# scychon/openmm_drudeNose

Measured on AMD Instinct MI355X. Metric: integrator steps/sec at 1M Drude pairs, higher is better.
Workload: dtype f64; 1 GPU; SWM4-NDP water box, 1000000 molecules = 5000000 particle slots, 1000000 Drude pairs, 1 temperature group (+ molecular-COM and Drude thermostats), TGNH mode, mixed precision, numNHChains=1, hard wall 0.02 nm, harness force call-out inside the timed region (harness_force: lattice); harness_force=lattice, precision=mixed, variant=resident, hipgraph=False, parallelism=particle-sharded x1 (whole molecules), one KE all-reduce per step, slots_per_gpu=5000000

## Files before the change

include/drude_tgnh.h:

```cpp
#ifndef DRUDE_TGNH_H_
#define DRUDE_TGNH_H_

#include <stdint.h>

#ifdef __cplusplus
extern "C" {
#endif

#define TGNH_ABI_VERSION 1

typedef int tgnh_status;
enum {
    TGNH_OK = 0,
    TGNH_ERR_ARG = -1,
    TGNH_ERR_GROUP_MISMATCH = -2,
    TGNH_ERR_HARDWALL = -3,
    TGNH_ERR_UNSUPPORTED = -4,
    TGNH_ERR_HIP = -5,
    TGNH_ERR_STATE = -6
};

enum { TGNH_MODE_DUALNH = 0,
       TGNH_MODE_TGNH = 1 };

enum { TGNH_PREC_SINGLE = 0,
       TGNH_PREC_MIXED = 1,
       TGNH_PREC_DOUBLE = 2 };

enum { TGNH_FLAG_DEFER_SCALE = 2 };
enum { TGNH_FLAG_WAVE_TILES = 8 };
enum { TGNH_FLAG_RESIDENT_STEP = 4 };

enum { TGNH_FLAG_TRUST_STATE_CHANGED = 16 };

enum { TGNH_FLAG_GATHER = 32 };

typedef struct tgnh_desc {
    uint32_t struct_size;
    int32_t mode;
    int32_t precision;
    int32_t flags;
    int32_t device;
    int32_t num_particles;
    int32_t padded_num_particles;
    int32_t num_pairs;
    int32_t num_groups;
    int32_t num_residues;
    int32_t num_constraints;
    int32_t has_cm_motion_remover;
    const double* mass;
    const int32_t* pair_drude;
    const int32_t* pair_parent;
    const int32_t* group;
    const int32_t* resid;
    const int32_t* constraint_i;
    const int32_t* constraint_j;
    double kB;
    double temperature, coupling_time;
    double drude_temperature, drude_coupling_time;
    double step_size;
    int32_t drude_steps_per_real_step;
    int32_t num_nh_chains;
    int32_t use_drude_nh_chains;
    int32_t use_com_temp_group;
    double max_drude_distance;
} tgnh_desc;

typedef struct tgnh_context* tgnh_handle;


typedef int (*tgnh_allreduce_fn)(void* buf, int count, void* stream, void* user);

const char* tgnh_last_error(void);
int tgnh_abi_version(void);

tgnh_status tgnh_create(const tgnh_desc* desc, tgnh_handle* out);
tgnh_status tgnh_destroy(tgnh_handle h);

tgnh_status tgnh_bind_buffers(tgnh_handle h, void* posq, void* posq_correction, void* velm,
                              const void* force, void* pos_delta);

tgnh_status tgnh_set_step_size(tgnh_handle h, double dt);
tgnh_status tgnh_set_drude_steps_per_real_step(tgnh_handle h, int n);
tgnh_status tgnh_set_max_drude_distance(tgnh_handle h, double d);

tgnh_status tgnh_get_local_dof_terms(tgnh_handle h, double* terms, int* count);
tgnh_status tgnh_set_global_dof_terms(tgnh_handle h, const double* terms, int count);
tgnh_status tgnh_set_allreduce(tgnh_handle h, tgnh_allreduce_fn fn, void* user);

#define TGNH_RCCL_ID_BYTES 128
tgnh_status tgnh_rccl_unique_id(void* id_out);
tgnh_status tgnh_rccl_init(tgnh_handle h, int world, int rank, const void* id);
tgnh_status tgnh_set_rccl_comm(tgnh_handle h, void* nccl_comm);
tgnh_status tgnh_rccl_shutdown(tgnh_handle h);
tgnh_status tgnh_set_resident_share(tgnh_handle h, int share);
tgnh_status tgnh_get_resident_work_groups(tgnh_handle h, int* per_compute_unit);
tgnh_status tgnh_get_step_path(tgnh_handle h, int* gather, const char** reason);
tgnh_status tgnh_get_resident_kernel(tgnh_handle h, int* which);

#define TGNH_XCHG_HANDLE_BYTES 64
tgnh_status tgnh_exchange_create(tgnh_handle h, int world, int rank, void* ipc_handle_out, void** mailbox_out);
tgnh_status tgnh_exchange_attach(tgnh_handle h, const void* ipc_handles);
tgnh_status tgnh_exchange_attach_pointers(tgnh_handle h, void* const* mailboxes);
tgnh_status tgnh_exchange_detach(tgnh_handle h);
tgnh_status tgnh_exchange_wait_stats(tgnh_handle h, void* stream, double* mean_us, double* max_us, int64_t* exchanges);

tgnh_status tgnh_step_begin(tgnh_handle h, void* stream);
tgnh_status tgnh_step_end(tgnh_handle h, void* stream);
tgnh_status tgnh_step_begin_kick(tgnh_handle h, void* stream);
tgnh_status tgnh_step_begin_move(tgnh_handle h, void* stream);
tgnh_status tgnh_step_end_kick(tgnh_handle h, void* stream);
tgnh_status tgnh_step_end_thermo(tgnh_handle h, void* stream);
tgnh_status tgnh_flush(tgnh_handle h, void* stream);
tgnh_status tgnh_note_replayed_steps(tgnh_handle h, int nsteps);
tgnh_status tgnh_get_pending_state(tgnh_handle h, uint32_t* bits);
tgnh_status tgnh_set_time(tgnh_handle h, double time, int64_t step_count);
tgnh_status tgnh_state_changed(tgnh_handle h);

tgnh_status tgnh_get_kinetic_energy(tgnh_handle h, int ke_sum_valid, void* stream, double* out);
tgnh_status tgnh_get_num_thermostats(tgnh_handle h, int* count);
tgnh_status tgnh_get_last_kinetic_energies(tgnh_handle h, void* stream, double* ke);
tgnh_status tgnh_get_last_scale_factors(tgnh_handle h, void* stream, double* scale);
tgnh_status tgnh_get_status_flags(tgnh_handle h, void* stream, uint32_t* flags);
tgnh_status tgnh_get_time(tgnh_handle h, double* time, int64_t* step_count);
tgnh_status tgnh_get_dof(tgnh_handle h, double* dof, double* nkt);

tgnh_status tgnh_get_thermostat_len(tgnh_handle h, int which, int* len);
tgnh_status tgnh_get_thermostat_state(tgnh_handle h, int which, void* stream, double* out);
tgnh_status tgnh_set_thermostat_state(tgnh_handle h, int which, void* stream, const double* in);

tgnh_status tgnh_get_topology_len(tgnh_handle h, int which, int* len);
tgnh_status tgnh_get_topology(tgnh_handle h, int which, int32_t* out);
tgnh_status tgnh_get_launch_bounds(tgnh_handle h, int32_t out[8]);

tgnh_status tgnh_compute_kinetic_energies(tgnh_handle h, void* stream);
tgnh_status tgnh_half_kick(tgnh_handle h, void* stream);

tgnh_status tgnh_harness_force(tgnh_handle h, const void* x0, double k_drude, double k_tether,
                               void* force_out, void* stream);
tgnh_status tgnh_harness_pack_sites(tgnh_handle h, const void* x0);
tgnh_status tgnh_harness_lattice_hint(tgnh_handle h, int mol_slots, int side, double spacing, const double* geom, int first_molecule);
tgnh_status tgnh_harness_sites_kind(tgnh_handle h, int* kind);
tgnh_status tgnh_run_steps(tgnh_handle h, int nsteps, void* stream);
tgnh_status tgnh_run_harness(tgnh_handle h, const void* x0, double k_drude, double k_tether,
                             int nsteps, void* stream);

tgnh_status tgnh_harness_set_clusters(tgnh_handle h, int n, const int32_t* atoms, const double* dist);
tgnh_status tgnh_harness_shake_positions(tgnh_handle h, double tol, void* stream);
tgnh_status tgnh_harness_shake_velocities(tgnh_handle h, double tol, void* stream);
tgnh_status tgnh_harness_set_virtual_sites(tgnh_handle h, int n, const int32_t* atoms, const double* weights);
tgnh_status tgnh_harness_virtual_sites(tgnh_handle h, void* stream);
tgnh_status tgnh_run_harness_constrained(tgnh_handle h, const void* x0, double k_drude, double k_tether,
                                         double tol, int nsteps, void* stream);

tgnh_status tgnh_harness_water_force(tgnh_handle h, double box, double cutoff, void* force_out, void* stream);
tgnh_status tgnh_harness_remove_cm_motion(tgnh_handle h, void* stream);

tgnh_status tgnh_timing_enable(tgnh_handle h, int on);
tgnh_status tgnh_timing_read(tgnh_handle h, int kernel, double* total_ms, int64_t* launches);
tgnh_status tgnh_algorithmic_bytes(tgnh_handle h, int kernel, double* bytes);

#ifdef __cplusplus
}
#endif
#endif
```

openmm_drudenose_amd/_lib.py:

```python
import ctypes as C
import os

HERE = os.path.dirname(os.path.abspath(__file__))
LIB_PATH = os.environ.get("TGNH_LIB") or os.path.join(HERE, "libdrudetgnh_hip.so")

TGNH_OK = 0
ERR_ARG, ERR_GROUP_MISMATCH, ERR_HARDWALL, ERR_UNSUPPORTED, ERR_HIP, ERR_STATE = -1, -2, -3, -4, -5, -6
MODE_DUALNH, MODE_TGNH = 0, 1
PREC_SINGLE, PREC_MIXED, PREC_DOUBLE = 0, 1, 2
FLAG_DEFER_SCALE, FLAG_RESIDENT_STEP, FLAG_WAVE_TILES, FLAG_TRUST_STATE_CHANGED, FLAG_GATHER = 2, 4, 8, 16, 32
KID_SKD, KID_KICK_KE, KID_SCALE, KID_KE, KID_CHAIN, KID_FORCE, KID_OTHER, KID_STEP = range(8)
KERNEL_NAMES = {KID_SKD: "scale+kick+drift", KID_KICK_KE: "kick+KE", KID_SCALE: "rescale", KID_KE: "KE",
                KID_CHAIN: "chain", KID_FORCE: "harness force", KID_OTHER: "other", KID_STEP: "resident step"}

c_i32p = C.POINTER(C.c_int32)
c_f64p = C.POINTER(C.c_double)


class TgnhDesc(C.Structure):
    _fields_ = [
        ("struct_size", C.c_uint32), ("mode", C.c_int32), ("precision", C.c_int32), ("flags", C.c_int32),
        ("device", C.c_int32), ("num_particles", C.c_int32), ("padded_num_particles", C.c_int32),
        ("num_pairs", C.c_int32), ("num_groups", C.c_int32), ("num_residues", C.c_int32),
        ("num_constraints", C.c_int32), ("has_cm_motion_remover", C.c_int32),
        ("mass", c_f64p), ("pair_drude", c_i32p), ("pair_parent", c_i32p), ("group", c_i32p), ("resid", c_i32p),
        ("constraint_i", c_i32p), ("constraint_j", c_i32p),
        ("kB", C.c_double), ("temperature", C.c_double), ("coupling_time", C.c_double),
        ("drude_temperature", C.c_double), ("drude_coupling_time", C.c_double), ("step_size", C.c_double),
        ("drude_steps_per_real_step", C.c_int32), ("num_nh_chains", C.c_int32),
        ("use_drude_nh_chains", C.c_int32), ("use_com_temp_group", C.c_int32),
        ("max_drude_distance", C.c_double),
    ]


ALLREDUCE_FN = C.CFUNCTYPE(C.c_int, C.c_void_p, C.c_int, C.c_void_p, C.c_void_p)

SIGNATURES = {
    "tgnh_last_error": (C.c_char_p, []),
    "tgnh_abi_version": (C.c_int, []),
    "tgnh_create": (C.c_int, [C.POINTER(TgnhDesc), C.POINTER(C.c_void_p)]),
    "tgnh_destroy": (C.c_int, [C.c_void_p]),
    "tgnh_bind_buffers": (C.c_int, [C.c_void_p] * 6),
    "tgnh_set_step_size": (C.c_int, [C.c_void_p, C.c_double]),
    "tgnh_set_drude_steps_per_real_step": (C.c_int, [C.c_void_p, C.c_int]),
    "tgnh_set_max_drude_distance": (C.c_int, [C.c_void_p, C.c_double]),
    "tgnh_get_local_dof_terms": (C.c_int, [C.c_void_p, c_f64p, C.POINTER(C.c_int)]),
    "tgnh_set_global_dof_terms": (C.c_int, [C.c_void_p, c_f64p, C.c_int]),
    "tgnh_set_allreduce": (C.c_int, [C.c_void_p, ALLREDUCE_FN, C.c_void_p]),
    "tgnh_rccl_unique_id": (C.c_int, [C.c_void_p]),
    "tgnh_rccl_init": (C.c_int, [C.c_void_p, C.c_int, C.c_int, C.c_void_p]),
    "tgnh_set_rccl_comm": (C.c_int, [C.c_void_p, C.c_void_p]),
    "tgnh_rccl_shutdown": (C.c_int, [C.c_void_p]),
    "tgnh_exchange_wait_stats": (C.c_int, [C.c_void_p, C.c_void_p, c_f64p, c_f64p, C.POINTER(C.c_int64)]),
    "tgnh_get_pending_state": (C.c_int, [C.c_void_p, C.POINTER(C.c_uint32)]),
    "tgnh_set_resident_share": (C.c_int, [C.c_void_p, C.c_int]),
    "tgnh_get_resident_work_groups": (C.c_int, [C.c_void_p, C.POINTER(C.c_int)]),
    "tgnh_get_resident_kernel": (C.c_int, [C.c_void_p, C.POINTER(C.c_int)]),
    "tgnh_get_step_path": (C.c_int, [C.c_void_p, C.POINTER(C.c_int), C.POINTER(C.c_char_p)]),
    "tgnh_exchange_create": (C.c_int, [C.c_void_p, C.c_int, C.c_int, C.c_void_p, C.POINTER(C.c_void_p)]),
    "tgnh_exchange_attach": (C.c_int, [C.c_void_p, C.c_char_p]),
    "tgnh_exchange_attach_pointers": (C.c_int, [C.c_void_p, C.POINTER(C.c_void_p)]),
    "tgnh_exchange_detach": (C.c_int, [C.c_void_p]),
    "tgnh_step_begin": (C.c_int, [C.c_void_p, C.c_void_p]),
    "tgnh_step_end": (C.c_int, [C.c_void_p, C.c_void_p]),
    "tgnh_step_begin_kick": (C.c_int, [C.c_void_p, C.c_void_p]),
    "tgnh_step_begin_move": (C.c_int, [C.c_void_p, C.c_void_p]),
    "tgnh_step_end_kick": (C.c_int, [C.c_void_p, C.c_void_p]),
    "tgnh_step_end_thermo": (C.c_int, [C.c_void_p, C.c_void_p]),
    "tgnh_flush": (C.c_int, [C.c_void_p, C.c_void_p]),
    "tgnh_state_changed": (C.c_int, [C.c_void_p]),
    "tgnh_note_replayed_steps": (C.c_int, [C.c_void_p, C.c_int]),
    "tgnh_set_time": (C.c_int, [C.c_void_p, C.c_double, C.c_int64]),
    "tgnh_get_kinetic_energy": (C.c_int, [C.c_void_p, C.c_int, C.c_void_p, c_f64p]),
    "tgnh_get_num_thermostats": (C.c_int, [C.c_void_p, C.POINTER(C.c_int)]),
    "tgnh_get_last_kinetic_energies": (C.c_int, [C.c_void_p, C.c_void_p, c_f64p]),
    "tgnh_get_last_scale_factors": (C.c_int, [C.c_void_p, C.c_void_p, c_f64p]),
    "tgnh_get_status_flags": (C.c_int, [C.c_void_p, C.c_void_p, C.POINTER(C.c_uint32)]),
    "tgnh_get_time": (C.c_int, [C.c_void_p, c_f64p, C.POINTER(C.c_int64)]),
    "tgnh_get_dof": (C.c_int, [C.c_void_p, c_f64p, c_f64p]),
    "tgnh_get_thermostat_len": (C.c_int, [C.c_void_p, C.c_int, C.POINTER(C.c_int)]),
    "tgnh_get_thermostat_state": (C.c_int, [C.c_void_p, C.c_int, C.c_void_p, c_f64p]),
    "tgnh_set_thermostat_state": (C.c_int, [C.c_void_p, C.c_int, C.c_void_p, c_f64p]),
    "tgnh_get_topology_len": (C.c_int, [C.c_void_p, C.c_int, C.POINTER(C.c_int)]),
    "tgnh_get_topology": (C.c_int, [C.c_void_p, C.c_int, c_i32p]),
    "tgnh_get_launch_bounds": (C.c_int, [C.c_void_p, c_i32p]),
    "tgnh_compute_kinetic_energies": (C.c_int, [C.c_void_p, C.c_void_p]),
    "tgnh_half_kick": (C.c_int, [C.c_void_p, C.c_void_p]),
    "tgnh_harness_force": (C.c_int, [C.c_void_p, C.c_void_p, C.c_double, C.c_double, C.c_void_p, C.c_void_p]),
    "tgnh_harness_pack_sites": (C.c_int, [C.c_void_p, C.c_void_p]),
    "tgnh_harness_lattice_hint": (C.c_int, [C.c_void_p, C.c_int, C.c_int, C.c_double, c_f64p, C.c_int]),
    "tgnh_harness_sites_kind": (C.c_int, [C.c_void_p, C.POINTER(C.c_int)]),
    "tgnh_run_harness": (C.c_int, [C.c_void_p, C.c_void_p, C.c_double, C.c_double, C.c_int, C.c_void_p]),
    "tgnh_run_steps": (C.c_int, [C.c_void_p, C.c_int, C.c_void_p]),
    "tgnh_harness_set_clusters": (C.c_int, [C.c_void_p, C.c_int, c_i32p, c_f64p]),
    "tgnh_harness_shake_positions": (C.c_int, [C.c_void_p, C.c_double, C.c_void_p]),
    "tgnh_harness_shake_velocities": (C.c_int, [C.c_void_p, C.c_double, C.c_void_p]),
    "tgnh_harness_set_virtual_sites": (C.c_int, [C.c_void_p, C.c_int, c_i32p, c_f64p]),
    "tgnh_harness_virtual_sites": (C.c_int, [C.c_void_p, C.c_void_p]),
    "tgnh_run_harness_constrained": (C.c_int, [C.c_void_p, C.c_void_p, C.c_double, C.c_double, C.c_double, C.c_int, C.c_void_p]),
    "tgnh_harness_water_force": (C.c_int, [C.c_void_p, C.c_double, C.c_double, C.c_void_p, C.c_void_p]),
    "tgnh_harness_remove_cm_motion": (C.c_int, [C.c_void_p, C.c_void_p]),
    "tgnh_timing_enable": (C.c_int, [C.c_void_p, C.c_int]),
    "tgnh_timing_read": (C.c_int, [C.c_void_p, C.c_int, c_f64p, C.POINTER(C.c_int64)]),
    "tgnh_algorithmic_bytes": (C.c_int, [C.c_void_p, C.c_int, c_f64p]),
}

_lib = None


def load():
    global _lib
    if _lib is not None:
        return _lib
    if not os.path.exists(LIB_PATH):
        raise RuntimeError(
            f"{LIB_PATH} is missing: build it with `python -m openmm_drudenose_amd.build` "
            "(hipcc --offload-arch=gfx950). There is no CPU fallback for the integrator path.")
    try:
        import torch
    except ImportError:
        pass
    lib = C.CDLL(LIB_PATH)
    for name, (res, args) in SIGNATURES.items():
        if os.environ.get("TGNH_LIB") and not hasattr(lib, name):
            continue
        fn = getattr(lib, name)
        fn.restype = res
        fn.argtypes = args
    _lib = lib
    return lib
```

openmm_drudenose_amd/csrc/tgnh_context.h:

```cpp
#ifndef TGNH_CONTEXT_H_
#define TGNH_CONTEXT_H_

#include <map>
#include <string>
#include <vector>

#include "tgnh_internal.h"

void tgnh_set_error(const std::string& msg);

namespace tgnh {
template <typename T> class DeviceBuf {
    T* p_ = nullptr;
    bool pinned_ = false;
public:
    DeviceBuf() = default;
    DeviceBuf(DeviceBuf&& o) noexcept : p_(o.p_), pinned_(o.pinned_) { o.p_ = nullptr; }
    ~DeviceBuf() { reset(); }
    void reset() { if (p_) (void)(pinned_ ? hipHostFree(p_) : hipFree(p_)); p_ = nullptr; }
    hipError_t alloc(size_t n, bool zero = false, unsigned ext_flags = 0) {
        reset(); pinned_ = false;
        void* p = nullptr;
        hipError_t e = ext_flags ? hipExtMallocWithFlags(&p, sizeof(T) * n, ext_flags) : hipMalloc(&p, sizeof(T) * n);
        if (e != hipSuccess) return e;
        p_ = static_cast<T*>(p);
        return zero ? hipMemset(p_, 0, sizeof(T) * n) : hipSuccess;
    }
    hipError_t alloc_pinned(size_t n) { reset(); pinned_ = true; return hipHostMalloc(reinterpret_cast<void**>(&p_), sizeof(T) * n, hipHostMallocDefault); }
    hipError_t upload(const T* src, size_t n) {
        hipError_t e = alloc(n ? n : 1);
        return e != hipSuccess || !n ? e : hipMemcpy(p_, src, sizeof(T) * n, hipMemcpyHostToDevice);
    }
    hipError_t upload(const std::vector<T>& v) { return upload(v.data(), v.size()); }
    T* get() const { return p_; }
    operator T*() const { return p_; }
};
typedef DeviceBuf<unsigned char> DeviceBytes;
}

struct tgnh_context {
    tgnh_desc d;
    int device = 0;
    bool host_only = false;
    struct Topology {
        std::vector<double> mass;
        std::vector<int> pair_drude, pair_parent, group, resid, normal;
        std::vector<int> res_count, res_first;
        std::vector<int> tile_start, tile_res;
        std::vector<int2> res_entries;
        std::vector<int> big_first, big_count;
        int num_big = 0, num_tiles = 0;
        std::vector<uint32_t> meta;
        std::vector<int2> wave_tile;
        std::vector<uint32_t> wmeta;
        std::vector<uint32_t> tile_pat, wtile_pat;
        std::vector<uint32_t> pattern, wpattern;
        int num_wtiles = 0;
        tgnh::DeviceBuf<uint32_t> d_meta, d_wmeta, d_tile_pat, d_pattern, d_wpattern;
        tgnh::DeviceBuf<int> d_tile_start, d_tile_res;
        tgnh::DeviceBuf<int2> d_res_table, d_wave_tile, d_big_table;
        tgnh::DeviceBytes d_big_com;
    } topo;
    struct Gather {
        bool generic = false;
        bool chain = false;
        std::string reason;
        std::vector<int2> res_table;
        std::vector<int> resid, partner;
        int com_lanes = 64;
        tgnh::DeviceBuf<int> d_group, d_resid, d_partner;
        tgnh::DeviceBuf<int2> d_res_table;
        tgnh::DeviceBytes d_com;
        tgnh::DeviceBuf<double> d_scratch;
    } gather;
    struct Thermostat {
        std::vector<double> h_state;
        std::vector<double> local_terms, global_terms;
        std::vector<double> dof, nkbt;
        double realkbT = 0, drudekbT = 0;
        tgnh::ChainLayout L{};
        tgnh::DeviceBuf<double> d_partials;
        tgnh::DeviceBuf<double> d_state;
        tgnh::DeviceBuf<double> d_stage;
        tgnh::DeviceBuf<double> d_scalar;
    } thermo;
    struct LaunchConfig {
        int grid = 0, gb = 1;
        int num_cus = 256, grid_override = 0;
        std::map<int, int> grid_cache;
        bool alternate_sweeps = true;
        int inline_sum_rows = tgnh::CHAIN_INLINE_SUM_ROWS;
        bool inline_sum_all = false;
        bool carry_ok = false;
        bool inline_chain = false;
        bool wave_ke = false;
        int resident_grid[5][2] = {{0, 0}, {0, 0}, {0, 0}, {0, 0}, {0, 0}};
        int resident_share = 1;
        int wresident_per_cu = 0, wresident_grid = 0;
        int resident_per_cu = 0;
    } cfg;
    struct Owed {
        bool end_pending = false;
        bool scale_pending = false;
        bool kick_pending = false;
        bool first_half_done = false;
        bool chain_pending = false;
        bool sum_pending = false;
        bool xwait_pending = false;
        bool stage_pending = false;
        bool ke_carry = false;
        bool chain_pending_twice = false;
        bool carry_pending = false;
        bool tail_summed = false;
        bool end_folded = false;
        bool g_com_fresh = false;
        enum : uint32_t { BIT_SWEEP_REVERSE = 1u << 8 };
        uint32_t bits() const {
            return end_pending | scale_pending << 1 | kick_pending << 2 | first_half_done << 3 | chain_pending << 4 | sum_pending << 5 |
                   xwait_pending << 6 | stage_pending << 7 | ke_carry << 9;
        }
        void chain_ran() { chain_pending = sum_pending = xwait_pending = carry_pending = false; }
        void velocities_current() { scale_pending = kick_pending = false; }
        void end_half_deferred(bool kick) { scale_pending = first_half_done = true; kick_pending = kick; }
        void resident_settled() { end_pending = first_half_done = false; velocities_current(); chain_pending = sum_pending = xwait_pending = false; }
        void thermostat_reset() { end_pending = first_half_done = false; velocities_current(); chain_pending = stage_pending = carry_pending = ke_carry = false; }
    } owed;
    struct Run {
        double time = 0;
        int64_t step_count = 0;
        int sweep_reverse = 0;
        int ke_parts = 0;
    } run;
    struct Bound {
        void *posq = nullptr, *posq_corr = nullptr, *velm = nullptr, *pos_delta = nullptr;
        const void* force = nullptr;
    } bound;
    struct Status {
        tgnh::DeviceBuf<uint32_t> d_word;
        tgnh::DeviceBuf<uint32_t> h_seen;
        int failed_code = 0;
        std::string failed;
    } status;
    struct Meeting {
        tgnh::DeviceBuf<unsigned int> d_sync;
        tgnh::DeviceBuf<unsigned long long> d_rows;
        tgnh::DeviceBuf<unsigned long long> self_box;
        tgnh::DeviceBuf<unsigned long long> d_self_misc;
        tgnh::XchgArgs self_x{};
    } meet;
    struct Exchange {
        tgnh_allreduce_fn allreduce = nullptr;
        void* allreduce_user = nullptr;
        void* rccl_comm = nullptr;
        bool rccl_owned = false;
        tgnh::XchgArgs args{};
        bool on = false;
        int world = 0, rank = 0;
        tgnh::DeviceBuf<unsigned long long> mailbox;
        tgnh::DeviceBuf<unsigned long long*> d_peers;
        std::vector<void*> opened;
        tgnh::DeviceBuf<unsigned long long> d_seq;
        tgnh::DeviceBuf<unsigned int> d_dead;
        tgnh::DeviceBuf<unsigned long long> d_stat;
        void close_peers() { for (void* p : opened) (void)hipIpcCloseMemHandle(p); opened.clear(); }
        ~Exchange() { close_peers(); }
    } xchg;
    struct Harness {
        tgnh::DeviceBuf<int4> d_cl_atoms, d_vs_atoms;
        tgnh::DeviceBuf<double> d_cl_dist, d_vs_w;
        int num_clusters = 0, num_sites = 0;
        tgnh::DeviceBuf<uint8_t> d_sflag;
        tgnh::DeviceBuf<uint32_t> d_sbase;
        tgnh::DeviceBytes d_sites;
        int lat_k = 0, lat_side = 0, lat_mol0 = 0;
        double lat_spacing = 0;
        std::vector<double> lat_geom;
        bool lat_on = false;
        tgnh::DeviceBuf<unsigned char> d_lat_tab;
        tgnh::DeviceBytes d_g_x0;
    } harness;
    struct Timing {
        bool on = false;
        int only = -1;
        struct Ev { hipEvent_t a, b; int kid; };
        std::vector<Ev> ev_pool;
        size_t ev_used = 0;
        double t_total[tgnh::KID_COUNT] = {0};
        int64_t t_count[tgnh::KID_COUNT] = {0};
        ~Timing() { for (auto& e : ev_pool) { (void)hipEventDestroy(e.a); (void)hipEventDestroy(e.b); } }
    } timing;
};

#endif
```

openmm_drudenose_amd/csrc/tgnh_internal.h:

```cpp
#ifndef TGNH_INTERNAL_H_
#define TGNH_INTERNAL_H_

#include <hip/hip_runtime.h>
#include <stdint.h>

#include "../../include/drude_tgnh.h"

namespace tgnh {

#ifndef TGNH_SPT
#define TGNH_SPT 2
#endif
#ifndef TGNH_TBLOCK
#define TGNH_TBLOCK 256
#endif
constexpr int BLOCK = 256;
constexpr int TBLOCK = TGNH_TBLOCK;
constexpr int SPT = TGNH_SPT;
constexpr int TILE_SLOTS = TBLOCK * SPT;
constexpr int TILE_RES = TILE_SLOTS / 2;
constexpr int GRID_CAP = 2048;
constexpr int MAX_GROUPS = 32;

constexpr uint32_t ROLE_NORMAL = 0, ROLE_DRUDE = 1, ROLE_PARENT = 2;
inline uint32_t pack_meta(uint32_t role, uint32_t group, int partner_off, uint32_t local_res) {
    return role | (group << 2) | ((uint32_t)(partner_off + 1024) << 10) | (local_res << 21);
}

constexpr int WAVE_SLOTS = 64;
constexpr int WBLOCK = 512;
inline uint32_t pack_wmeta(uint32_t role, uint32_t group, int partner_off, uint32_t pos_in_mol, uint32_t mol_slots_m1) {
    return role | (group << 2) | ((uint32_t)(partner_off + 64) << 10) | (pos_in_mol << 17) | (mol_slots_m1 << 23);
}

constexpr int PATTERN_WORDS = 64;

enum : int {
    OP_SCALE = 1,
    OP_KICK = 2,
    OP_DRIFT = 4,
    OP_KE = 8,
    OP_POSDELTA = 16,
    OP_MOVE = 32,
    OP_PREKICK = 64,
    OP_NOSTORE = 128
};

enum : int { KID_SKD = 0, KID_KICK_KE = 1, KID_SCALE = 2, KID_KE = 3, KID_CHAIN = 4, KID_FORCE = 5,
             KID_OTHER = 6, KID_STEP = 7, KID_COUNT = 8 };

struct ChainLayout {
    int mode, G, NT, C, use_drude_chains;
    int len_eta, len_etaDot, len_etaDotDot, len_etaMass;
    int off_eta, off_etaDot, off_etaDotDot, off_etaMass;
    int off_nkbt;
    int off_ke;
    int off_ke_red;
    int off_scale;
    int off_scale_a;
    int off_scale_b;
    int off_kesum;
    int off_ke_post;
    int total;
    int numTempGroup, idxMaxNHChains, iNumNHChains;
    int c1_shift, c1_mul, c1_add, c1_unused, c1_guard_below;
    int c1_quirk;
};

constexpr int XCHG_NT_PAD = 40;
constexpr int XCHG_CELL_U64 = 2;
constexpr int XCHG_MAX_WORLD = 16;
constexpr unsigned XCHG_SPIN_LIMIT = 1000000u;
constexpr unsigned CENSUS_SPIN_LIMIT = 20000u;
#ifndef TGNH_XCHG_REPLICAS
#define TGNH_XCHG_REPLICAS 32
#endif
constexpr int XCHG_REPLICAS = TGNH_XCHG_REPLICAS;
constexpr size_t XCHG_REPLICA_U64 =
    ((sizeof(unsigned long long) * 2 * (size_t)XCHG_MAX_WORLD * XCHG_NT_PAD * XCHG_CELL_U64 + 4095) / 4096 * 4096 + 256) / sizeof(unsigned long long);
constexpr size_t XCHG_MAILBOX_BYTES(int ) { return sizeof(unsigned long long) * XCHG_REPLICA_U64 * XCHG_REPLICAS; }

struct XchgArgs {
    int on;
    int world, rank;
    unsigned long long* const* peers;
    unsigned long long* mine;
    unsigned long long* seq;
    unsigned int* dead;
    unsigned int* status;
    unsigned long long* stat;
};

constexpr int CHAIN_INLINE_SUM_NT = 10;
constexpr int CHAIN_INLINE_SUM_ROWS = 256;

struct ChainArgs {
    ChainLayout L;
    XchgArgs x;
    int x_send, x_wait;
    double* st;
    uint32_t* status;
    const double* partials;
    int nparts;
    int nbig;
    const double* stage;
    int commit;
    int do_sum;
    int do_chain;
    int chain_twice;
    int lanes;
    int ke_carry;
    double dt;
    int S;
    double dtc, inv_dtc;
    double realkbT, drudekbT;
};

struct TileArgs {
    void* posq;
    void* posq_corr;
    void* velm;
    const long long* force;
    void* pos_delta;
    const uint32_t* meta;
    const int* tile_start;
    const int* tile_res;
    const int2* res_table;
    const void* big_com;
    const double* scale;
    double* partials;
    uint32_t* status;
    unsigned int* sync;
    int census;
    unsigned long long* rows;
    const int2* wave_tile;
    const uint32_t* wmeta;
    const uint32_t* tile_pat;
    const uint32_t* pattern;
    const uint32_t* wpattern;
    int num_wtiles;
    int tail_sum;
    double* ke_red;
    int num_tiles;
    int reverse;
    int padded;
    int num_groups;
    int use_com;
    int hardwall;
    double dt;
    double max_dist;
    double hw_scale;
    int chain_on;
    int sum_rows;
    int commit_len, commit_skip, commit_skip_n;
    const double* commit_src;
    double* commit_dst;
    int x_wait;
    const double* st_in;
    double* st_out;
    ChainArgs chain;
};

struct BigComArgs {
    const int2* table;
    int n;
    const void* velm;
    const long long* force;
    int padded;
    int kick;
    double dt;
    void* big_com;
    double* partials;
    int NT, G;
};

struct ForceArgs {
    const void* posq;
    const void* posq_corr;
    const void* x0;
    const uint32_t* meta;
    long long* force;
    int n, padded;
    int reverse;
    double k_drude, k_tether;
    const uint8_t* sflag;
    const uint32_t* sbase;
    const void* sites;
    int lat_k, lat_side, lat_mol0;
    double lat_spacing, lat_inv_k, lat_inv_side, lat_inv_side2;
    const unsigned char* lat_tab;
};
constexpr size_t LAT_TAB_BYTES = 64 + 64 * 3 * sizeof(double);

constexpr int GATHER_KE_ROWS = 1024;
constexpr int GATHER_MAX_NT = 2048;
struct GatherArgs {
    void* posq; void* posq_corr; void* velm; const long long* force; void* pos_delta;
    const int* group;
    const int* resid;
    const int2* res_table;
    const int* partner;
    void* com;
    const double* scale;
    double* partials;
    uint32_t* status;
    int n, padded, n_res, G, NT, use_com, hardwall, ops, kick_com;
    int com_lanes;
    double dt, max_dist, hw_scale;
};

#define TGNH_LAUNCH(...) do { (void)hipGetLastError(); hipLaunchKernelGGL(__VA_ARGS__); } while (0)

hipError_t launch_tile(int precision, int ops, int gb, const TileArgs& a, int grid, size_t lds, hipStream_t s);
int tile_blocks_per_cu(int precision, int ops, int gb, size_t lds, bool multi = false);
hipError_t launch_step(int precision, int gb, int kind, const TileArgs& a, int grid, size_t lds, hipStream_t s);
int step_blocks_per_cu(int precision, int gb, int kind, size_t lds);
int step_kind_ops2(int kind);
hipError_t launch_wstep(int precision, int gb, bool multi, const TileArgs& a, int grid, hipStream_t s);
int wstep_blocks_per_cu(int precision, int gb, bool multi);
hipError_t launch_wke(int precision, int ops, int gb, const TileArgs& a, int grid, hipStream_t s);
int wke_blocks_per_cu(int precision, int ops, int gb);
hipError_t launch_chain(const ChainArgs& a, hipStream_t s);
hipError_t launch_big_com(int precision, const BigComArgs& a, hipStream_t s);
hipError_t launch_force(int precision, const ForceArgs& a, hipStream_t s);
hipError_t launch_gather_com(int precision, const GatherArgs& a, hipStream_t s);
int gather_ke_grid(const GatherArgs& a);
hipError_t launch_gather_ke(int precision, const GatherArgs& a, int grid, hipStream_t s);
hipError_t launch_gather_rowsum(const double* partials, int nrows, int NT, double* ke_red, hipStream_t s);
hipError_t launch_gather_chain(const ChainArgs& a, double* scratch, hipStream_t s);
hipError_t launch_gather_update(int precision, const GatherArgs& a, hipStream_t s);
hipError_t launch_gather_force(int precision, const GatherArgs& a, const void* x0, long long* force, double k_drude, double k_tether, hipStream_t s);
constexpr int PLAIN_KE_PARTS = 2048;
hipError_t launch_plain_ke(int precision, const void* velm, const long long* force, int n, int padded,
                           double time_shift, double* out , hipStream_t s);
size_t tile_lds_bytes(int precision, int ops, bool hardwall, bool use_com);

}

#endif
```

openmm_drudenose_amd/csrc/tgnh_kernels.hip:

```cpp
#include "tgnh_tile_device.h"

#ifdef TGNH_TRACE
TGNH_TRACE_READERS(tgnh_debug_read_trace, tgnh_debug_clear_trace)
extern "C" int tgnh_debug_read_chain_trace(unsigned long long* out) {
    return (int)hipMemcpyFromSymbol(out, HIP_SYMBOL(tgnh::g_chain_trace), sizeof(unsigned long long) * 8);
}
#endif

namespace tgnh {


size_t tile_lds_bytes(int precision, int ops, bool hardwall, bool use_com) {
    (void)use_com;
    const size_t m4 = (precision == TGNH_PREC_SINGLE) ? 16 : 32;
    const bool hw = hardwall && (ops & (OP_DRIFT | OP_MOVE));
    size_t b = (size_t)(TBLOCK / 64) * (MAX_GROUPS + 2) * 8;
    if ((ops & (OP_SCALE | OP_KE)) || hw) b = m4 * (TILE_SLOTS + TILE_RES);
    if (hw) b += m4 * TILE_SLOTS;
    return b;
}

#ifndef TGNH_MINWAVES
#define TGNH_MINWAVES 1
#endif
// ... 644 lines not shown
    auto load = [&](const Bounds& b, WaveIn<PREC>& in) {
        const bool patterned = pw.of(a, (uint32_t)b.y >> 8, lane);
        wave_load<PREC, OPS>(a, b.ws, b.n, patterned, pw.word, lane, in);
    };
    if (w < nw) { bounds(w, b0); load(b0, A); }
    if (w + stride < nw) bounds(w + stride, b1);
    while (w < nw) {
        if (w + 2 * stride < nw) bounds(w + 2 * stride, b2);
        if (w + stride < nw) load(b1, B);
        work(A, b0);
        w += stride;
        if (w >= nw) break;
        if (w + 2 * stride < nw) bounds(w + 2 * stride, b0);
        if (w + stride < nw) load(b2, A);
        work(B, b1);
        w += stride;
        b1 = b0; b0 = b2;
    }
#pragma unroll
    for (int b = 0; b < GB; b++) ke_g[b] = wave_sum(ke_g[b]);
    ke_com = wave_sum(ke_com);
    ke_drude = wave_sum(ke_drude);
    if (lane == 0) {
#pragma unroll
        for (int b = 0; b < GB; b++) sred[wv][b] = ke_g[b];
        sred[wv][GB] = ke_com;
        sred[wv][GB + 1] = ke_drude;
    }
    __syncthreads();
    if (tid < GB + 2) {
        double t = 0.0;
#pragma unroll
        for (int k = 0; k < TBLOCK / 64; k++) t += sred[k][tid];
        const int b = tid < GB ? tid : G + (tid - GB);
        if (tid >= GB || tid < G) {
            if (a.tail_sum) {
                unsigned long long* cell = a.rows + row_word((int)blockIdx.x, 2 * b);
                const unsigned long long bits = (unsigned long long)__double_as_longlong(t), tg = (unsigned long long)(gen0 + 1u) << 32;
                __hip_atomic_store(cell, tg | (bits & 0xffffffffull), __ATOMIC_RELAXED, __HIP_MEMORY_SCOPE_SYSTEM);
                __hip_atomic_store(cell + 64, tg | (bits >> 32), __ATOMIC_RELAXED, __HIP_MEMORY_SCOPE_SYSTEM);
            } else a.partials[(size_t)blockIdx.x * (G + 2) + b] = t;
        }
    }
    if (a.tail_sum && blockIdx.x == 0) {
        __shared__ double s_tail[TBLOCK / 64][GB + 2];
        const int NT = G + 2;
        double acc[GB + 2];
#pragma unroll
        for (int b = 0; b < GB + 2; b++) acc[b] = 0.0;
        const bool ok = collect_rows<GB, false, TBLOCK>(a, tid, (int)gridDim.x, NT, (unsigned long long)(gen0 + 1u), acc);
        if (!ok) atomicOr(a.status, 16u);
#pragma unroll
        for (int b = 0; b < GB + 2; b++) {
            if (b < NT) {
                const double t = wave_sum(acc[b]);
                if (lane == 0) s_tail[wv][b] = t;
            }
        }
        const bool all_ok = __syncthreads_and(ok ? 1 : 0) != 0;
        if (tid < NT) {
            double t = 0.0;
#pragma unroll
            for (int k = 0; k < TBLOCK / 64; k++) t += s_tail[k][tid];
            a.ke_red[tid] = all_ok ? t : __longlong_as_double(0x7ff8000000000000ll);
        }
        if (tid == 0) a.sync[1] = gen0 + 1u;
    }
}



enum : int { STEP_DEFER = 0, STEP_PLAIN_BEGIN = 1, STEP_PLAIN_END = 2, STEP_SPLIT_BEGIN = 3, STEP_SPLIT_END = 4, STEP_KINDS = 5 };
constexpr int step_ops1(int kind) {
    return (kind == STEP_DEFER || kind == STEP_PLAIN_END) ? (OP_KICK | OP_KE | OP_NOSTORE) : OP_KE;
}
constexpr int step_ops2(int kind) {
    return kind == STEP_DEFER ? (OP_PREKICK | OP_SCALE | OP_KICK | OP_DRIFT)
         : kind == STEP_PLAIN_BEGIN ? (OP_SCALE | OP_KICK | OP_DRIFT)
         : kind == STEP_PLAIN_END ? (OP_PREKICK | OP_SCALE)
         : kind == STEP_SPLIT_BEGIN ? (OP_SCALE | OP_KICK | OP_POSDELTA)
         : OP_SCALE;
}

template <int PREC, int GB, int KIND>
__global__ __launch_bounds__(TBLOCK, TGNH_MINWAVES) void step_kernel(const TileArgs a) {
    typedef typename Prec<PREC>::mixed mixed;
    constexpr int STEP_OPS1 = step_ops1(KIND), STEP_OPS2 = step_ops2(KIND);
    __shared__ double s_scale[MAX_GROUPS + 2];
    __shared__ double s_part[TBLOCK / 64][CHAIN_INLINE_SUM_NT];
    __shared__ double s_x[64 + XCHG_MAX_WORLD * CHAIN_INLINE_SUM_NT];
    __shared__ int s_go;
    __shared__ unsigned s_gen;
    __shared__ unsigned long long s_seq1;
    extern __shared__ __attribute__((aligned(16))) char smem[];
    const int tid = threadIdx.x, G = a.num_groups, NT = G + 2;
    const int grid = (int)gridDim.x;
    const bool chain_wave = tid < 64;
    const int itg = tid & 63;
    if (a.census) {
        if (tid == 0) {
            __hip_atomic_fetch_add(&a.sync[2], 1u, __ATOMIC_RELAXED, __HIP_MEMORY_SCOPE_AGENT);
            unsigned n = 0;
            while (__hip_atomic_load(&a.sync[2], __ATOMIC_RELAXED, __HIP_MEMORY_SCOPE_AGENT) < gridDim.x && ++n < CENSUS_SPIN_LIMIT)
                __builtin_amdgcn_s_sleep(16);
            if (__hip_atomic_load(&a.sync[2], __ATOMIC_RELAXED, __HIP_MEMORY_SCOPE_AGENT) < gridDim.x) atomicOr(&a.sync[3], 1u);
        }
        return;
    }
    TileEnv<PREC, GB> e;
    e.init(a, smem, s_scale, OpsOf<STEP_OPS2>::POS && a.hardwall != 0);
    auto tile_of = [&](int tt) { return a.reverse ? a.num_tiles - 1 - tt : tt; };

    unsigned gen0 = 0;
    unsigned long long seq0 = 0;
    Chain1Regs creg{};
    if (chain_wave) {
        gen0 = __hip_atomic_load(&a.sync[1], __ATOMIC_RELAXED, __HIP_MEMORY_SCOPE_AGENT);
        seq0 = __hip_atomic_load(a.chain.x.seq, __ATOMIC_RELAXED, __HIP_MEMORY_SCOPE_AGENT);
        if (itg < NT) creg = chain1_load(a.chain, a.st_in, itg);
    }

    TRACE(0);
    TileIn<PREC> cur;
    int tt = blockIdx.x;
    TilePattern tp;
    tile_load<PREC, STEP_OPS1>(a, tile_of(tt), cur, tp);
    for (;;) {
        tile_body<PREC, STEP_OPS1, GB>(a, e, cur, 4);
        if (tt + grid >= a.num_tiles) break;
        tt += grid;
        tile_load<PREC, STEP_OPS1>(a, tile_of(tt), cur, tp);
    }
    const int tt_last = tt;
    TRACE(1);
    MeetShared sh{s_scale, s_part, s_x, &s_go, &s_gen, &s_seq1, nullptr};
    if (!step_meet<PREC, GB>(a, e, gen0, seq0, creg, sh, [&] { tile_load<PREC, STEP_OPS2, STEP_OPS1>(a, tile_of(tt_last), cur, tp); }))
        return;
    e.s_com = (mixed)s_scale[G]; e.s_drude = (mixed)s_scale[G + 1];
    TRACE(9);

    tt = tt_last;
    for (bool held = true;; held = false) {
        tile_body<PREC, STEP_OPS2, GB>(a, e, cur, 0, held);
        if (tt - grid < 0) break;
        tt -= grid;
        tile_load<PREC, STEP_OPS2>(a, tile_of(tt), cur, tp);
    }
    TRACE(15);
}


template <int PREC, int GB, bool MULTI = false>
__global__ __launch_bounds__(WBLOCK) void wstep_kernel(const TileArgs a) {
    typedef typename Prec<PREC>::mixed mixed;
    static_assert(GB > 0, "register bins only");
    __shared__ double s_scale[MAX_GROUPS + 2];
    __shared__ double s_part[WBLOCK / 64][CHAIN_INLINE_SUM_NT];
    __shared__ double s_x[64 + XCHG_MAX_WORLD * CHAIN_INLINE_SUM_NT];
    __shared__ int s_go;
    __shared__ unsigned s_gen;
    __shared__ unsigned long long s_seq1;
    __shared__ mixed s_img[WBLOCK / 64][7][WAVE_SLOTS];
    __shared__ double s_block[256];
    const int tid = threadIdx.x, lane = tid & 63, G = a.num_groups, NT = G + 2;
    const int wv = __builtin_amdgcn_readfirstlane(tid >> 6);
    const bool chain_wave = tid < 64;
    const int itg = tid & 63;
    if (a.census) {
        if (tid == 0) {
            __hip_atomic_fetch_add(&a.sync[2], 1u, __ATOMIC_RELAXED, __HIP_MEMORY_SCOPE_AGENT);
            unsigned n = 0;
            while (__hip_atomic_load(&a.sync[2], __ATOMIC_RELAXED, __HIP_MEMORY_SCOPE_AGENT) < gridDim.x && ++n < CENSUS_SPIN_LIMIT)
                __builtin_amdgcn_s_sleep(16);
            if (__hip_atomic_load(&a.sync[2], __ATOMIC_RELAXED, __HIP_MEMORY_SCOPE_AGENT) < gridDim.x) atomicOr(&a.sync[3], 1u);
        }
        return;
    }
    TileEnv<PREC, GB> e;
    e.tid = tid; e.G = G; e.smem = nullptr; e.wbins0 = nullptr; e.s_scale = s_scale;
    e.clear_ke();
    WaveStep<PREC, GB> ws(a, &e, s_scale, &s_img[wv][0][0], lane);
    typedef WaveBounds Bounds;
    auto bounds = [&](const int ww, Bounds& b) { ws.bounds(ww, b); };
    auto load_vf = [&](const Bounds& b, WStepIn<PREC>& in) { ws.load_vf(b, in); };
    auto load_x = [&](const Bounds& b, WStepIn<PREC>& in) { ws.load_x(b, in); };
    auto prepare = [&](WStepIn<PREC>& t, const Bounds& bd, const bool ke) { ws.template prepare<true>(t, bd, ke); };
    auto finish = [&](WStepIn<PREC>& t, const Bounds& bd) { ws.finish(t, bd); };
    auto wfence = [] { WaveStep<PREC, GB>::wfence(); };

    unsigned gen0 = 0;
    unsigned long long seq0 = 0;
    Chain1Regs creg{};
    if (chain_wave) {
        gen0 = __hip_atomic_load(&a.sync[1], __ATOMIC_RELAXED, __HIP_MEMORY_SCOPE_AGENT);
        seq0 = __hip_atomic_load(a.chain.x.seq, __ATOMIC_RELAXED, __HIP_MEMORY_SCOPE_AGENT);
        if (itg < NT && !(MULTI && a.chain.L.C > 1)) creg = chain1_load(a.chain, a.st_in, itg);
    }
    if (MULTI && a.chain.L.C > 1 && tid < a.chain.L.total) s_block[tid] = a.st_in[tid];

    const int nw = a.num_wtiles, stride = (int)gridDim.x * (WBLOCK / 64);

    TRACE(0);
    const int w0 = __builtin_amdgcn_readfirstlane((int)blockIdx.x * (WBLOCK / 64) + wv);
    const bool have = w0 < nw;
    int w = w0;
    Bounds b0{}, b1{};
    WStepIn<PREC> cur;
    if (have) {
        bounds(w, b0);
        if (w + stride < nw) bounds(w + stride, b1);
        load_vf(b0, cur);
    }
    while (have) {
#ifdef TGNH_TRACE
        if (w == w0) { asm volatile("s_waitcnt vmcnt(0)" ::: "memory"); TRACE(3); }
#endif
        prepare(cur, b0, true);
#ifdef TGNH_TRACE
        if (w == w0) TRACE(4);
#endif
        if (w + stride >= nw) break;
        wfence();
        w += stride;
        b0 = b1;
        if (w + stride < nw) bounds(w + stride, b1);
        load_vf(b0, cur);
    }
    const int w_last = w;
    TRACE(1);
    MeetShared sh{s_scale, s_part, s_x, &s_go, &s_gen, &s_seq1, s_block};
    if (!step_meet<PREC, GB, true, WBLOCK, MULTI>(a, e, gen0, seq0, creg, sh, [&] {
            if (have) {
                load_x(b0, cur);
                if (w_last - stride >= 0) bounds(w_last - stride, b1);
            }
        })) return;

    TRACE(9);
    if (have) {
        w = w_last;
        finish(cur, b0);
        TRACE(5);
        while (w - stride >= 0) {
            w -= stride;
            b0 = b1;
            if (w - stride >= 0) bounds(w - stride, b1);
            load_vf(b0, cur); load_x(b0, cur);
            prepare(cur, b0, false);
            finish(cur, b0);
        }
    }
    TRACE(15);
}

constexpr int CHAIN_LDS_DOUBLES = 2048;

__device__ __forceinline__ void chain_prologue(const ChainArgs& a, double (*sred)[MAX_GROUPS + 2], double* s_chain, double* s_ke) {
    const ChainLayout& L = a.L;
    const int NT = L.NT, tid = threadIdx.x, lane = tid & 63, wv = tid >> 6;
    double* st = a.st;
    if (a.commit) {
        for (int i = tid; i < L.total; i += BLOCK)
            if (i < L.off_ke_red || i >= L.off_ke_red + NT) st[i] = a.stage[i];
        __syncthreads();
    }
    if (a.do_sum) {
        constexpr int PER = GRID_CAP / BLOCK;
        double acc[MAX_GROUPS + 2];
#pragma unroll
        for (int b = 0; b < MAX_GROUPS + 2; b++) acc[b] = 0.0;
        if (NT <= 4) {
            double val[PER][4];
#pragma unroll
            for (int j = 0; j < PER; j++) {
                const int p = tid + j * BLOCK;
#pragma unroll
                for (int b = 0; b < 4; b++) val[j][b] = (p < a.nparts && b < NT) ? a.partials[(size_t)p * NT + b] : 0.0;
            }
#pragma unroll
            for (int j = 0; j < PER; j++)
#pragma unroll
                for (int b = 0; b < 4; b++) acc[b] += val[j][b];
        } else {
#pragma unroll
            for (int b = 0; b < MAX_GROUPS + 2; b++) {
                if (b < NT) {
                    double val[PER];
#pragma unroll
                    for (int j = 0; j < PER; j++) { const int p = tid + j * BLOCK; val[j] = p < a.nparts ? a.partials[(size_t)p * NT + b] : 0.0; }
#pragma unroll
                    for (int j = 0; j < PER; j++) acc[b] += val[j];
                }
            }
        }
        for (int p = tid; p < a.nbig; p += BLOCK) {
#pragma unroll
            for (int b = 0; b < MAX_GROUPS + 2; b++)
                if (b < NT) acc[b] += a.partials[((size_t)GRID_CAP + p) * NT + b];
        }
#pragma unroll
        for (int b = 0; b < MAX_GROUPS + 2; b++) {
            if (b < NT) {
                const double s = wave_sum(acc[b]);
                if (lane == 0) sred[wv][b] = s;
            }
        }
        __syncthreads();
        if (tid < NT) {
            double s = 0.0;
            for (int w = 0; w < BLOCK / 64; w++) s += sred[w][tid];
            st[L.off_ke_red + tid] = s;
            s_ke[tid] = s;
        }
        __syncthreads();
    } else if (tid < NT) {
        s_ke[tid] = st[chain_ke_src(a) + tid];
    }
    if (tid < NT && a.status && !a.ke_carry && s_ke[tid] != s_ke[tid]) atomicOr(a.status, 16u);
    if (a.x_send) xchg_send(a.x, NT, tid, BLOCK, s_chain, tid < NT ? s_ke[tid] : 0.0);
    if (a.x_wait) {
        __syncthreads();
        if (tid < 64) {
            const double tot = xchg_wait_sum(a.x, NT, tid, s_chain);
            if (tid < NT) { s_ke[tid] = tot; st[L.off_ke_red + tid] = tot; }
        }
        __syncthreads();
    }
}

__global__ __launch_bounds__(BLOCK) void rowsum_kernel(const ChainArgs a) {
    __shared__ double sred[BLOCK / 64][MAX_GROUPS + 2];
    __shared__ double s_chain[2 * XCHG_MAX_WORLD * XCHG_NT_PAD > 64 ? 2 * XCHG_MAX_WORLD * XCHG_NT_PAD : 64];
    __shared__ double s_ke[MAX_GROUPS + 2];
    chain_prologue(a, sred, s_chain, s_ke);
}

__global__ __launch_bounds__(BLOCK) void chain_kernel(const ChainArgs a) {
    __shared__ double sred[BLOCK / 64][MAX_GROUPS + 2];
    __shared__ double s_chain[CHAIN_LDS_DOUBLES];
    __shared__ double s_ke[MAX_GROUPS + 2];
    const ChainLayout& L = a.L;
    const int NT = L.NT, tid = threadIdx.x;
    double* st = a.st;
    CHAIN_TRACE(0);
    chain_prologue(a, sred, s_chain, s_ke);
    if (!a.do_chain) return;
    if (!a.do_sum) __syncthreads();
    CHAIN_TRACE(1);
    if (L.mode == TGNH_MODE_TGNH && L.C > 4 && L.C <= 16 && a.lanes) {
        chain_lanes_run(a, st, tid, BLOCK, s_ke);
        if (tid == 0) {
            double s = 0.0;
            for (int i = 0; i < NT; i++) s += s_ke[i];
            st[L.off_kesum] = 0.5 * s;
        }
    } else if (L.mode == TGNH_MODE_TGNH) {
        int itg = -1;
        if (tid < NT - 1) itg = tid;
        else if (tid == 64) itg = NT - 1;
        if (itg >= 0) {
            switch (L.C) {
                case 1: { Chain1Regs r = chain1_load(a, a.st, itg); r.ke = s_ke[itg]; chain1_run(a, r, a.st, true, nullptr, itg); } break;
                case 2: run_tgnh<2>(a, a.st, a.st, true, nullptr, itg, s_chain, s_ke[itg]); break;
                case 3: run_tgnh<3>(a, a.st, a.st, true, nullptr, itg, s_chain, s_ke[itg]); break;
                case 4: run_tgnh<4>(a, a.st, a.st, true, nullptr, itg, s_chain, s_ke[itg]); break;
                default: run_tgnh<0>(a, a.st, a.st, true, nullptr, itg, s_chain, s_ke[itg]); break;
            }
        }
        if (tid == 0) {
            double s = 0.0;
            for (int i = 0; i < NT; i++) s += s_ke[i];
            st[L.off_kesum] = 0.5 * s;
        }
    } else if (L.C == 1) {
        if (tid < 3) {
            Chain1Regs r = chain1_load(a, a.st, tid); r.ke = s_ke[tid];
            if (L.c1_quirk) chain1q_run(a, r, a.st, true, nullptr, tid);
            else chain1_run(a, r, a.st, true, nullptr, tid);
        }
        if (tid == 64) st[L.off_kesum] = 0.5 * (s_ke[0] + s_ke[2]);
    } else if (tid == 0) {
        switch (L.C) {
            case 1: run_dualnh<1>(a, a.st, a.st, true, nullptr, s_chain, s_ke[0], s_ke[1], s_ke[2]); break;
            case 2: run_dualnh<2>(a, a.st, a.st, true, nullptr, s_chain, s_ke[0], s_ke[1], s_ke[2]); break;
            case 3: run_dualnh<3>(a, a.st, a.st, true, nullptr, s_chain, s_ke[0], s_ke[1], s_ke[2]); break;
            case 4: run_dualnh<4>(a, a.st, a.st, true, nullptr, s_chain, s_ke[0], s_ke[1], s_ke[2]); break;
            default: run_dualnh<0>(a, a.st, a.st, true, nullptr, s_chain, s_ke[0], s_ke[1], s_ke[2]); break;
        }
    }
    CHAIN_TRACE(2);
}
template <int CC>
__global__ __launch_bounds__(BLOCK) void chain_long_kernel(const ChainArgs a) {
    __shared__ double sred[BLOCK / 64][MAX_GROUPS + 2];
    __shared__ double s_chain[2 * XCHG_MAX_WORLD * XCHG_NT_PAD > 64 ? 2 * XCHG_MAX_WORLD * XCHG_NT_PAD : 64];
    __shared__ double s_ke[MAX_GROUPS + 2];
    const ChainLayout& L = a.L;
    const int NT = L.NT, tid = threadIdx.x;
    chain_prologue(a, sred, s_chain, s_ke);
    if (!a.do_sum) __syncthreads();
    int itg = -1;
    if (tid < NT - 1) itg = tid;
    else if (tid == 64) itg = NT - 1;
    if (itg >= 0) run_tgnh<CC>(a, a.st, a.st, true, nullptr, itg, nullptr, s_ke[itg]);
    if (tid == 0) {
// ... 152 lines not shown
    if ((threadIdx.x & 63) == 0) sred[threadIdx.x >> 6] = e;
    __syncthreads();
    if (threadIdx.x == 0) {
        double s = 0.0;
        for (int w = 0; w < BLOCK / 64; w++) s += sred[w];
        out[1 + blockIdx.x] = s;
    }
}

__global__ __launch_bounds__(BLOCK) void plain_ke_sum_kernel(double* out, int nparts) {
    __shared__ double sred[BLOCK / 64];
    double e = 0.0;
    for (int i = threadIdx.x; i < nparts; i += BLOCK) e += out[1 + i];
    e = wave_sum(e);
    if ((threadIdx.x & 63) == 0) sred[threadIdx.x >> 6] = e;
    __syncthreads();
    if (threadIdx.x == 0) {
        double s = 0.0;
        for (int w = 0; w < BLOCK / 64; w++) s += sred[w];
        out[0] = 0.5 * s;
    }
}

typedef void (*tile_fn_t)(const TileArgs);

template <int PREC, int OPS>
static tile_fn_t tile_fn_gb(int gb) {
    if constexpr ((OPS & OP_KE) != 0) {
        if (gb == 0) return tile_kernel<PREC, OPS, 0>;
        if (gb <= 1) return tile_kernel<PREC, OPS, 1>;
        if (gb <= 4) return tile_kernel<PREC, OPS, 4>;
        return tile_kernel<PREC, OPS, 8>;
    } else {
        return tile_kernel<PREC, OPS, 1>;
    }
}

template <int PREC>
static tile_fn_t tile_fn_ops(int ops, int gb) {
    switch (ops) {
        case OP_KE: return tile_fn_gb<PREC, OP_KE>(gb);
        case OP_SCALE: return tile_fn_gb<PREC, OP_SCALE>(gb);
        case OP_SCALE | OP_KICK | OP_DRIFT: return tile_fn_gb<PREC, OP_SCALE | OP_KICK | OP_DRIFT>(gb);
        case OP_KICK | OP_KE: return tile_fn_gb<PREC, OP_KICK | OP_KE>(gb);
        case OP_KICK | OP_KE | OP_NOSTORE: return tile_fn_gb<PREC, OP_KICK | OP_KE | OP_NOSTORE>(gb);
        case OP_PREKICK | OP_SCALE | OP_KICK | OP_DRIFT: return tile_fn_gb<PREC, OP_PREKICK | OP_SCALE | OP_KICK | OP_DRIFT>(gb);
        case OP_PREKICK | OP_SCALE: return tile_fn_gb<PREC, OP_PREKICK | OP_SCALE>(gb);
        case OP_KICK: return tile_fn_gb<PREC, OP_KICK>(gb);
        case OP_SCALE | OP_KICK | OP_POSDELTA: return tile_fn_gb<PREC, OP_SCALE | OP_KICK | OP_POSDELTA>(gb);
        case OP_MOVE: return tile_fn_gb<PREC, OP_MOVE>(gb);
        default: return nullptr;
    }
}

static tile_fn_t tile_fn(int precision, int ops, int gb) {
    switch (precision) {
        case TGNH_PREC_SINGLE: return tile_fn_ops<TGNH_PREC_SINGLE>(ops, gb);
        case TGNH_PREC_MIXED: return tile_fn_ops<TGNH_PREC_MIXED>(ops, gb);
        case TGNH_PREC_DOUBLE: return tile_fn_ops<TGNH_PREC_DOUBLE>(ops, gb);
        default: return nullptr;
    }
}

template <int PREC> static tile_fn_t tile_fn_multi(int ops) {
    switch (ops) {
        case OP_SCALE: return tile_kernel<PREC, OP_SCALE, 1, true>;
        case OP_SCALE | OP_KICK | OP_DRIFT: return tile_kernel<PREC, OP_SCALE | OP_KICK | OP_DRIFT, 1, true>;
        case OP_PREKICK | OP_SCALE | OP_KICK | OP_DRIFT: return tile_kernel<PREC, OP_PREKICK | OP_SCALE | OP_KICK | OP_DRIFT, 1, true>;
        case OP_PREKICK | OP_SCALE: return tile_kernel<PREC, OP_PREKICK | OP_SCALE, 1, true>;
        case OP_SCALE | OP_KICK | OP_POSDELTA: return tile_kernel<PREC, OP_SCALE | OP_KICK | OP_POSDELTA, 1, true>;
        default: return nullptr;
    }
}
static tile_fn_t tile_fn_any(int precision, int ops, int gb, bool multi) {
    if (!multi) return tile_fn(precision, ops, gb);
    switch (precision) {
        case TGNH_PREC_SINGLE: return tile_fn_multi<TGNH_PREC_SINGLE>(ops);
        case TGNH_PREC_MIXED: return tile_fn_multi<TGNH_PREC_MIXED>(ops);
        case TGNH_PREC_DOUBLE: return tile_fn_multi<TGNH_PREC_DOUBLE>(ops);
        default: return nullptr;
    }
}

hipError_t launch_tile(int precision, int ops, int gb, const TileArgs& a, int grid, size_t lds, hipStream_t s) {
    tile_fn_t fn = tile_fn_any(precision, ops, gb, a.chain_on && a.chain.L.C > 1);
    if (!fn) return hipErrorInvalidValue;
    TGNH_LAUNCH(fn, dim3(grid), dim3(TBLOCK), lds, s, a);
    return hipGetLastError();
}

template <int PREC, int OPS> static tile_fn_t wke_fn_gb(int gb) {
    if (gb <= 1) return wke_kernel<PREC, OPS, 1>;
    if (gb <= 4) return wke_kernel<PREC, OPS, 4>;
    return wke_kernel<PREC, OPS, 8>;
}
template <int PREC> static tile_fn_t wke_fn_ops(int ops, int gb) {
    switch (ops) {
        case OP_KE: return wke_fn_gb<PREC, OP_KE>(gb);
        case OP_KICK | OP_KE: return wke_fn_gb<PREC, OP_KICK | OP_KE>(gb);
        case OP_KICK | OP_KE | OP_NOSTORE: return wke_fn_gb<PREC, OP_KICK | OP_KE | OP_NOSTORE>(gb);
        default: return nullptr;
    }
}
static tile_fn_t wke_fn(int precision, int ops, int gb) {
    if (gb == 0) return nullptr;
    switch (precision) {
        case TGNH_PREC_SINGLE: return wke_fn_ops<TGNH_PREC_SINGLE>(ops, gb);
        case TGNH_PREC_MIXED: return wke_fn_ops<TGNH_PREC_MIXED>(ops, gb);
        case TGNH_PREC_DOUBLE: return wke_fn_ops<TGNH_PREC_DOUBLE>(ops, gb);
        default: return nullptr;
    }
}
hipError_t launch_wke(int precision, int ops, int gb, const TileArgs& a, int grid, hipStream_t s) {
    tile_fn_t fn = wke_fn(precision, ops, gb);
    if (!fn) return hipErrorInvalidValue;
    TGNH_LAUNCH(fn, dim3(grid), dim3(TBLOCK), 0, s, a);
    return hipGetLastError();
}
int wke_blocks_per_cu(int precision, int ops, int gb) {
    tile_fn_t fn = wke_fn(precision, ops, gb);
    int n = 0;
    if (!fn || hipOccupancyMaxActiveBlocksPerMultiprocessor(&n, reinterpret_cast<const void*>(fn), TBLOCK, 0) != hipSuccess) return 0;
    return n;
}

typedef void (*step_fn_t)(const TileArgs);
template <int PREC, int KIND> static step_fn_t step_fn_gb(int gb) {
    if (gb <= 1) return step_kernel<PREC, 1, KIND>;
    if (gb <= 4) return step_kernel<PREC, 4, KIND>;
    return step_kernel<PREC, 8, KIND>;
}
template <int PREC> static step_fn_t step_fn_kind(int kind, int gb) {
    switch (kind) {
        case STEP_DEFER: return step_fn_gb<PREC, STEP_DEFER>(gb);
        case STEP_PLAIN_BEGIN: return step_fn_gb<PREC, STEP_PLAIN_BEGIN>(gb);
        case STEP_PLAIN_END: return step_fn_gb<PREC, STEP_PLAIN_END>(gb);
        case STEP_SPLIT_BEGIN: return step_fn_gb<PREC, STEP_SPLIT_BEGIN>(gb);
        case STEP_SPLIT_END: return step_fn_gb<PREC, STEP_SPLIT_END>(gb);
        default: return nullptr;
    }
}
static step_fn_t step_fn(int precision, int gb, int kind) {
    if (gb == 0) return nullptr;
    switch (precision) {
        case TGNH_PREC_SINGLE: return step_fn_kind<TGNH_PREC_SINGLE>(kind, gb);
        case TGNH_PREC_MIXED: return step_fn_kind<TGNH_PREC_MIXED>(kind, gb);
        case TGNH_PREC_DOUBLE: return step_fn_kind<TGNH_PREC_DOUBLE>(kind, gb);
        default: return nullptr;
    }
}
template <int PREC, bool MULTI> static step_fn_t wstep_fn_gb(int gb) {
    return gb <= 1 ? wstep_kernel<PREC, 1, MULTI> : gb <= 4 ? wstep_kernel<PREC, 4, MULTI> : wstep_kernel<PREC, 8, MULTI>;
}
static step_fn_t wstep_fn(int precision, int gb, bool multi) {
    if (gb == 0) return nullptr;
    switch (precision) {
        case TGNH_PREC_SINGLE: return multi ? wstep_fn_gb<TGNH_PREC_SINGLE, true>(gb) : wstep_fn_gb<TGNH_PREC_SINGLE, false>(gb);
        case TGNH_PREC_MIXED: return multi ? wstep_fn_gb<TGNH_PREC_MIXED, true>(gb) : wstep_fn_gb<TGNH_PREC_MIXED, false>(gb);
        case TGNH_PREC_DOUBLE: return multi ? wstep_fn_gb<TGNH_PREC_DOUBLE, true>(gb) : wstep_fn_gb<TGNH_PREC_DOUBLE, false>(gb);
        default: return nullptr;
    }
}
hipError_t launch_wstep(int precision, int gb, bool multi, const TileArgs& a, int grid, hipStream_t s) {
    step_fn_t fn = wstep_fn(precision, gb, multi);
    if (!fn) return hipErrorInvalidValue;
    TGNH_LAUNCH(fn, dim3(grid), dim3(WBLOCK), 0, s, a);
    return hipGetLastError();
}
int wstep_blocks_per_cu(int precision, int gb, bool multi) {
    step_fn_t fn = wstep_fn(precision, gb, multi);
    int n = 0;
    if (!fn || hipOccupancyMaxActiveBlocksPerMultiprocessor(&n, reinterpret_cast<const void*>(fn), WBLOCK, 0) != hipSuccess) return 0;
    return n;
}
int step_kind_ops2(int kind) { return step_ops2(kind); }
hipError_t launch_step(int precision, int gb, int kind, const TileArgs& a, int grid, size_t lds, hipStream_t s) {
    step_fn_t fn = step_fn(precision, gb, kind);
    if (!fn) return hipErrorInvalidValue;
    TGNH_LAUNCH(fn, dim3(grid), dim3(TBLOCK), lds, s, a);
    return hipGetLastError();
}
int step_blocks_per_cu(int precision, int gb, int kind, size_t lds) {
    step_fn_t fn = step_fn(precision, gb, kind);
    int n = 0;
    if (!fn || hipOccupancyMaxActiveBlocksPerMultiprocessor(&n, reinterpret_cast<const void*>(fn), TBLOCK, lds) != hipSuccess) return 0;
    return n;
}

int tile_blocks_per_cu(int precision, int ops, int gb, size_t lds, bool multi) {
    tile_fn_t fn = tile_fn_any(precision, ops, gb, multi);
    int n = 0;
    if (!fn || hipOccupancyMaxActiveBlocksPerMultiprocessor(&n, reinterpret_cast<const void*>(fn), TBLOCK, lds) != hipSuccess) return 0;
    return n;
}

hipError_t launch_chain(const ChainArgs& a, hipStream_t s) {
    if (!a.do_chain) TGNH_LAUNCH(rowsum_kernel, dim3(1), dim3(BLOCK), 0, s, a);
    else if (a.L.mode == TGNH_MODE_TGNH && a.L.C > 4 && a.L.C <= 16 && !a.lanes) {
        switch (a.L.C) {
#define TGNH_LONG(c) case c: TGNH_LAUNCH(chain_long_kernel<c>, dim3(1), dim3(BLOCK), 0, s, a); break;
            TGNH_LONG(5) TGNH_LONG(6) TGNH_LONG(7) TGNH_LONG(8) TGNH_LONG(9) TGNH_LONG(10) TGNH_LONG(11) TGNH_LONG(12)
            TGNH_LONG(13) TGNH_LONG(14) TGNH_LONG(15) TGNH_LONG(16)
#undef TGNH_LONG
        }
    }
    else if (a.L.mode == TGNH_MODE_DUALNH && a.L.C > 4 && a.L.C <= 16) {
        switch (a.L.C) {
#define TGNH_DLONG(c) case c: TGNH_LAUNCH(chain_dualnh_long_kernel<c>, dim3(1), dim3(BLOCK), 0, s, a); break;
            TGNH_DLONG(5) TGNH_DLONG(6) TGNH_DLONG(7) TGNH_DLONG(8) TGNH_DLONG(9) TGNH_DLONG(10) TGNH_DLONG(11) TGNH_DLONG(12)
            TGNH_DLONG(13) TGNH_DLONG(14) TGNH_DLONG(15) TGNH_DLONG(16)
#undef TGNH_DLONG
        }
    }
    else TGNH_LAUNCH(chain_kernel, dim3(1), dim3(BLOCK), 0, s, a);
#ifdef TGNH_TUNING
    static const int again = getenv("TGNH_CHAIN_REPEAT") ? atoi(getenv("TGNH_CHAIN_REPEAT")) : 0;
    for (int r = 0; r < again && a.do_chain; r++) { ChainArgs b = a; b.do_sum = 0; b.commit = 0; b.x_send = 0; b.x_wait = 0; TGNH_LAUNCH(chain_kernel, dim3(1), dim3(BLOCK), 0, s, b); }
#endif
    return hipGetLastError();
}

template <int PREC>
__global__ __launch_bounds__(BLOCK) void force_packed_kernel(const ForceArgs a) {
    typedef typename Prec<PREC>::real real;
    typedef typename Prec<PREC>::real4 real4;
    typedef typename Prec<PREC>::mixed mixed;
    const real4* __restrict__ posq = reinterpret_cast<const real4*>(a.posq);
    const float4* __restrict__ pcorr = reinterpret_cast<const float4*>(a.posq_corr);
    const real* __restrict__ sites = reinterpret_cast<const real*>(a.sites);
    const mixed kd = (mixed)a.k_drude, kt = (mixed)a.k_tether;
    const int lane = threadIdx.x & 63;
    const int nround = (a.n + gridDim.x * BLOCK - 1) / (gridDim.x * BLOCK);
    for (int rr = 0; rr < nround; rr++) {
        const int r = a.reverse ? nround - 1 - rr : rr;
        const int blk = a.reverse ? (int)gridDim.x - 1 - (int)blockIdx.x : (int)blockIdx.x;
        const int i = (r * gridDim.x + blk) * BLOCK + threadIdx.x;
        const bool in = i < a.n;
        uint32_t b = 0;
        real4 p = {}; float4 c = {};
        if (in) {
            b = a.sflag[i];
            p = posq[i];
            if (PREC == TGNH_PREC_MIXED) c = pcorr[i];
        }
        const bool tethered = (b & 4u) != 0;
        const unsigned long long before = __ballot(tethered) & ((1ull << lane) - 1ull);
        real s0 = 0, s1 = 0, s2 = 0;
        if (tethered) {
            const real* rec = sites + 3 * (size_t)(a.sbase[i >> 6] + (uint32_t)__popcll(before));
            s0 = rec[0]; s1 = rec[1]; s2 = rec[2];
        }
        mixed x = p.x, y = p.y, z = p.z;
        if (PREC == TGNH_PREC_MIXED) { x += (mixed)c.x; y += (mixed)c.y; z += (mixed)c.z; }
        const uint32_t role = b & 3u;
        int off = (int)(b >> 3) - 16;
        if (in && (b >> 3) == 0) off = (int)((a.meta[i] >> 10) & 2047u) - 1024;
        const int pl = lane + off;
        const int src = (pl >= 0 && pl < 64) ? pl : lane;
        mixed ox = __shfl(x, src, 64), oy = __shfl(y, src, 64), oz = __shfl(z, src, 64);
        mixed fx = 0, fy = 0, fz = 0;
        if (in) {
            if (tethered) { fx = -kt * (x - (mixed)s0); fy = -kt * (y - (mixed)s1); fz = -kt * (z - (mixed)s2); }
            if (role != ROLE_NORMAL) {
                if (src != pl) {
                    const int j = i + off;
                    const real4 q = posq[j];
                    ox = q.x; oy = q.y; oz = q.z;
                    if (PREC == TGNH_PREC_MIXED) { const float4 cq = pcorr[j]; ox += (mixed)cq.x; oy += (mixed)cq.y; oz += (mixed)cq.z; }
                }
                const bool is_d = role == ROLE_DRUDE;
                const mixed sgn = is_d ? (mixed)-1 : (mixed)1;
                const mixed sx = is_d ? x - ox : ox - x, sy = is_d ? y - oy : oy - y, sz = is_d ? z - oz : oz - z;
                fx += sgn * kd * sx; fy += sgn * kd * sy; fz += sgn * kd * sz;
            }
            a.force[i] = (long long)(fx * (mixed)4294967296.0);
            a.force[i + a.padded] = (long long)(fy * (mixed)4294967296.0);
            a.force[i + 2 * a.padded] = (long long)(fz * (mixed)4294967296.0);
        }
    }
}

template <int PREC>
__global__ __launch_bounds__(BLOCK) void force_lattice_kernel(const ForceArgs a) {
    typedef typename Prec<PREC>::real real;
    typedef typename Prec<PREC>::real4 real4;
    typedef typename Prec<PREC>::mixed mixed;
    __shared__ double s_geom[64 * 3];
    __shared__ unsigned char s_flag[64];
    const real4* __restrict__ posq = reinterpret_cast<const real4*>(a.posq);
    const float4* __restrict__ pcorr = reinterpret_cast<const float4*>(a.posq_corr);
    if (threadIdx.x < 64) s_flag[threadIdx.x] = a.lat_tab[threadIdx.x];
    if (threadIdx.x < 192) s_geom[threadIdx.x] = reinterpret_cast<const double*>(a.lat_tab + 64)[threadIdx.x];
    __syncthreads();
    const mixed kd = (mixed)a.k_drude, kt = (mixed)a.k_tether;
    const int lane = threadIdx.x & 63;
    const int nround = (a.n + gridDim.x * BLOCK - 1) / (gridDim.x * BLOCK);
    for (int rr = 0; rr < nround; rr++) {
        const int r = a.reverse ? nround - 1 - rr : rr;
        const int blk = a.reverse ? (int)gridDim.x - 1 - (int)blockIdx.x : (int)blockIdx.x;
        const int i = (r * gridDim.x + blk) * BLOCK + threadIdx.x;
        const bool in = i < a.n;
        real4 p = {}; float4 c = {};
        if (in) {
            p = posq[i];
            if (PREC == TGNH_PREC_MIXED) c = pcorr[i];
        }
        const int mloc = (int)(((double)i + 0.5) * a.lat_inv_k), pos = in ? i - mloc * a.lat_k : 0;
        const int mol = a.lat_mol0 + mloc;
        const uint32_t b = in ? s_flag[pos] : 0u;
        const bool tethered = (b & 4u) != 0;
        real s0 = 0, s1 = 0, s2 = 0;
        if (tethered) {
            const int ix = (int)(((double)mol + 0.5) * a.lat_inv_side2), rem = mol - ix * a.lat_side * a.lat_side;
            const int iy = (int)(((double)rem + 0.5) * a.lat_inv_side), iz = rem - iy * a.lat_side;
            s0 = (real)__dadd_rn(__dmul_rn((double)ix, a.lat_spacing), s_geom[3 * pos]);
            s1 = (real)__dadd_rn(__dmul_rn((double)iy, a.lat_spacing), s_geom[3 * pos + 1]);
            s2 = (real)__dadd_rn(__dmul_rn((double)iz, a.lat_spacing), s_geom[3 * pos + 2]);
        }
        mixed x = p.x, y = p.y, z = p.z;
        if (PREC == TGNH_PREC_MIXED) { x += (mixed)c.x; y += (mixed)c.y; z += (mixed)c.z; }
        const uint32_t role = b & 3u;
        const int off = (int)(b >> 3) - 16;
        const int pl = lane + off;
// ... 80 lines not shown
```

openmm_drudenose_amd/csrc/tgnh_lifecycle.cpp:

```cpp
#include <memory>

#include "tgnh_host.h"
#ifndef TGNH_MEETING_MEM
#define TGNH_MEETING_MEM hipDeviceMallocFinegrained
#endif

static thread_local std::string g_err;
extern "C" const char* tgnh_last_error(void) { return g_err.c_str(); }
extern "C" int tgnh_abi_version(void) { return TGNH_ABI_VERSION; }

void tgnh_set_error(const std::string& msg) { g_err = msg; }

static tgnh_status validate_desc(const tgnh_desc* d, bool* long_chain) {
    if (d->struct_size != sizeof(tgnh_desc)) return fail(TGNH_ERR_ARG, "tgnh_desc size mismatch (ABI)");
    if (d->mode != TGNH_MODE_DUALNH && d->mode != TGNH_MODE_TGNH) return fail(TGNH_ERR_ARG, "bad mode");
    if (d->precision < TGNH_PREC_SINGLE || d->precision > TGNH_PREC_DOUBLE) return fail(TGNH_ERR_ARG, "bad precision");
    if (d->num_particles < 1 || d->num_pairs < 0 || !d->mass || (d->num_pairs && (!d->pair_drude || !d->pair_parent)))
        return fail(TGNH_ERR_ARG, "bad particle / pair arrays");
    if (d->padded_num_particles < d->num_particles) return fail(TGNH_ERR_ARG, "padded_num_particles < num_particles");
    if (d->num_constraints < 0) return fail(TGNH_ERR_ARG, "negative num_constraints");
    if (3LL * d->padded_num_particles > 2147483647LL)
        return fail(TGNH_ERR_UNSUPPORTED, "more than 715 827 882 padded particle slots: the index into the third force plane leaves 32 bits");
    if (d->num_nh_chains < 1 || d->drude_steps_per_real_step < 1) return fail(TGNH_ERR_ARG, "numNHChains and drudeStepsPerRealStep must be >= 1");
    if (d->mode == TGNH_MODE_TGNH && (d->num_groups < 1 || d->num_residues < 1 || !d->group || !d->resid))
        return fail(TGNH_ERR_ARG, "TGNH mode needs temperature groups and residues");
    if (!(d->max_drude_distance >= 0)) return fail(TGNH_ERR_ARG, "setMaxDrudeDistance: Distance cannot be negative");
    if (d->flags & ~(uint32_t)(TGNH_FLAG_DEFER_SCALE | TGNH_FLAG_RESIDENT_STEP | TGNH_FLAG_WAVE_TILES | TGNH_FLAG_TRUST_STATE_CHANGED | TGNH_FLAG_GATHER))
        return fail(TGNH_ERR_ARG, "unknown bits in tgnh_desc.flags (a newer header than this library?)");
    if (d->mode == TGNH_MODE_DUALNH && d->num_pairs == 0)
        return fail(TGNH_ERR_UNSUPPORTED, "dualNH mode needs at least one Drude pair (the Reference platform does too)");
    if (!(d->step_size > 0) || !std::isfinite(d->step_size)) return fail(TGNH_ERR_ARG, "step size must be positive");
    *long_chain = false;
    {
        const long need = d->mode == TGNH_MODE_TGNH ? (long)(d->num_groups + 2) * (4L * d->num_nh_chains + 1)
                                                    : 4L * (2L * d->num_nh_chains + 4);
        if (d->num_nh_chains > (d->mode == TGNH_MODE_TGNH ? 16 : 4) && need > 2048) {
            if (d->mode != TGNH_MODE_TGNH) return fail(TGNH_ERR_UNSUPPORTED, "numNHChains too large for the on-device chain");
            *long_chain = true;
        }
    }
    return TGNH_OK;
}

static tgnh_status decide_policy(tgnh_context* c, const tgnh_desc* d, bool long_chain) {
    if (c->gather.generic) {
        c->d.flags &= ~(TGNH_FLAG_DEFER_SCALE | TGNH_FLAG_RESIDENT_STEP | TGNH_FLAG_TRUST_STATE_CHANGED | TGNH_FLAG_WAVE_TILES);
        c->gather.chain = c->d.mode == TGNH_MODE_TGNH && (c->thermo.L.NT > MAX_GROUPS + 2 || long_chain);
    }
    c->cfg.wave_ke = !c->gather.generic && !c->topo.wave_tile.empty() && c->cfg.gb != 0 &&
                 ((d->flags & TGNH_FLAG_WAVE_TILES) || (double)d->num_particles >= 0.9 * WAVE_SLOTS * (double)c->topo.num_wtiles);
#ifdef TGNH_TUNING
    if (const char* e = getenv("TGNH_WAVE_KE")) c->cfg.wave_ke = c->cfg.wave_ke && e[0] != '0';
#endif
    {
        bool inside = true;
        if (d->mode == TGNH_MODE_TGNH && d->use_com_temp_group) {
            std::vector<int> g0(d->num_residues, -1);
            for (int i = 0; i < d->num_particles && inside; i++) {
                if (c->topo.mass[i] == 0.0) continue;
                int& g = g0[c->topo.resid[i]];
                if (g == -1) g = c->topo.group[i];
                else if (g != c->topo.group[i]) inside = false;
            }
        }
        if ((c->d.flags & TGNH_FLAG_DEFER_SCALE) && !inside) return fail(TGNH_ERR_UNSUPPORTED, "DEFER_SCALE needs every molecule inside one temperature group");
        c->cfg.carry_ok = (c->d.flags & TGNH_FLAG_TRUST_STATE_CHANGED) && !(c->d.flags & TGNH_FLAG_DEFER_SCALE) && inside;
    }
    c->cfg.grid = GRID_CAP;
#ifdef TGNH_TUNING
    if (const char* e = getenv("TGNH_GRID")) { int g = atoi(e); if (g >= 1) c->cfg.grid_override = std::min(g, GRID_CAP); }
#endif
    {
        bool want = true;
        c->cfg.inline_sum_all = d->num_particles < 2000000;
#ifdef TGNH_TUNING
        if (const char* e = getenv("TGNH_INLINE_CHAIN")) want = e[0] != '0';
        if (const char* e4 = getenv("TGNH_INLINE_SUM_ROWS")) c->cfg.inline_sum_rows = atoi(e4);
        if (const char* e5 = getenv("TGNH_INLINE_SUM_ALL")) c->cfg.inline_sum_all = e5[0] != '0';
        if (const char* e3 = getenv("TGNH_ALTERNATE_SWEEPS")) c->cfg.alternate_sweeps = e3[0] != '0';
#endif
        int inline_multi_max = 2500000;
#ifdef TGNH_TUNING
        if (const char* e6 = getenv("TGNH_INLINE_MULTI_MAX")) inline_multi_max = atoi(e6);
#endif
        c->cfg.inline_chain = want && !c->gather.generic && (c->thermo.L.C == 1 || (c->thermo.L.C <= 4 && d->num_particles < inline_multi_max));
        if (c->thermo.L.total > 256 && c->thermo.L.C > 1) c->cfg.inline_chain = c->cfg.inline_chain && false;
    }
    return TGNH_OK;
}

static tgnh_status allocate(tgnh_context* c) {
    const size_t NT = c->thermo.L.NT;
    HIP_OK(c->thermo.d_partials.alloc((size_t)(c->cfg.grid + c->topo.num_big) * NT, true));
    HIP_OK(c->thermo.d_state.alloc(c->thermo.L.total));
    HIP_OK(c->thermo.d_stage.alloc(c->thermo.L.total));
    HIP_OK(c->status.d_word.alloc(1, true));
    HIP_OK(c->status.h_seen.alloc_pinned(1));
    *c->status.h_seen = 0;
    if (c->gather.chain && c->thermo.L.C > 4) HIP_OK(c->gather.d_scratch.alloc(NT * (4 * c->thermo.L.C + 1)));
    HIP_OK(c->thermo.d_scalar.alloc(1 + PLAIN_KE_PARTS));
    HIP_OK(c->meet.d_sync.alloc(4, true));
    const bool resident = (c->d.flags & TGNH_FLAG_RESIDENT_STEP) != 0;
    if (c->cfg.wave_ke || resident)
        HIP_OK(c->meet.d_rows.alloc(2 * (size_t)GRID_CAP * CHAIN_INLINE_SUM_NT, true, TGNH_MEETING_MEM));
    if (!resident) return TGNH_OK;
    HIP_OK(c->meet.self_box.alloc(XCHG_MAILBOX_BYTES(1) / sizeof(unsigned long long), true, TGNH_MEETING_MEM));
    HIP_OK(c->meet.d_self_misc.alloc(4, true));
    unsigned long long* const box = c->meet.self_box;
    HIP_OK(hipMemcpy(c->meet.d_self_misc + 2, &box, sizeof(box), hipMemcpyHostToDevice));
    c->meet.self_x = XchgArgs{};
    c->meet.self_x.on = 1; c->meet.self_x.world = 1; c->meet.self_x.rank = 0;
    c->meet.self_x.peers = reinterpret_cast<unsigned long long* const*>(c->meet.d_self_misc + 2);
    c->meet.self_x.mine = c->meet.self_box;
    c->meet.self_x.seq = c->meet.d_self_misc;
    c->meet.self_x.dead = reinterpret_cast<unsigned int*>(c->meet.d_self_misc + 1);
    c->meet.self_x.status = c->status.d_word;
    return TGNH_OK;
}

template <typename Launch> static tgnh_status census(tgnh_context* c, int per_cu_max, Launch&& launch, int* found) {
    for (int per_cu = std::min(per_cu_max, 8); per_cu >= 1 && !*found; per_cu--) {
        TileArgs a{};
        a.census = 1; a.sync = c->meet.d_sync;
        HIP_OK(hipMemset(c->meet.d_sync + 2, 0, 2 * sizeof(unsigned int)));
        const int grid = std::min(per_cu * c->cfg.num_cus, GRID_CAP);
        HIP_OK(launch(a, grid));
        unsigned int res[2] = {0, 1};
        HIP_OK(hipMemcpy(res, c->meet.d_sync + 2, sizeof(res), hipMemcpyDeviceToHost));
        if (res[0] == (unsigned)grid && res[1] == 0) *found = per_cu;
    }
    return TGNH_OK;
}

static tgnh_status resident_census(tgnh_context* c) {
    if (!(c->d.flags & TGNH_FLAG_RESIDENT_STEP) || c->cfg.gb == 0 || !c->cfg.inline_chain || c->thermo.L.NT > CHAIN_INLINE_SUM_NT) return TGNH_OK;
    const int kind = (c->d.flags & TGNH_FLAG_DEFER_SCALE) ? 0 : 1;
    const size_t lds = tile_lds_bytes(c->d.precision, step_kind_ops2(kind), true, true);
    tgnh_status rc = census(c, c->thermo.L.C == 1 ? step_blocks_per_cu(c->d.precision, c->cfg.gb, kind, lds) : 0,
                            [&](const TileArgs& a, int grid) { return launch_step(c->d.precision, c->cfg.gb, kind, a, grid, lds, (hipStream_t)0); },
                            &c->cfg.resident_per_cu);
    if (rc) return rc;
    const bool multi = c->thermo.L.C > 1;
    bool want_w = c->cfg.wave_ke && (c->d.flags & TGNH_FLAG_DEFER_SCALE) && (c->cfg.resident_per_cu > 0 || multi);
    if (c->d.mode == TGNH_MODE_DUALNH && !c->thermo.L.use_drude_chains && multi) want_w = false;
#ifdef TGNH_TUNING
    if (const char* e = getenv("TGNH_WSTEP")) want_w = want_w && e[0] != '0';
#endif
    return census(c, want_w ? wstep_blocks_per_cu(c->d.precision, c->cfg.gb, multi) : 0,
                  [&](const TileArgs& a, int grid) { return launch_wstep(c->d.precision, c->cfg.gb, multi, a, grid, (hipStream_t)0); },
                  &c->cfg.wresident_per_cu);
}

extern "C" tgnh_status tgnh_create(const tgnh_desc* d, tgnh_handle* out) {
    if (!d || !out) return fail(TGNH_ERR_ARG, "null argument");
    bool long_chain = false;
    tgnh_status rc = validate_desc(d, &long_chain); if (rc) return rc;
    const bool host_only = d->device == -1;
    if (!host_only) {
        int ndev = 0;
        HIP_OK(hipGetDeviceCount(&ndev));
        if (d->device < 0 || d->device >= ndev) return fail(TGNH_ERR_HIP, "no such HIP device (the HIP path needs an MI355X; there is no CPU fallback)");
        HIP_OK(hipSetDevice(d->device));
    }

    std::unique_ptr<tgnh_context> owner(new tgnh_context());
    tgnh_context* c = owner.get();
    c->host_only = host_only;
    c->d = *d;
    c->device = d->device;
    c->thermo.realkbT = d->kB * d->temperature;
    c->thermo.drudekbT = d->kB * d->drude_temperature;
    make_layout(c);
    c->cfg.gb = c->thermo.L.G <= 1 ? 1 : (c->thermo.L.G <= 4 ? 4 : (c->thermo.L.G <= 8 ? 8 : 0));
    if (long_chain) { c->gather.generic = true; c->gather.reason = "a chain too long for the LDS-resident form"; }
    else if (d->flags & TGNH_FLAG_GATHER) { c->gather.generic = true; c->gather.reason = "asked for (TGNH_FLAG_GATHER)"; }
    if (!host_only) {
        hipDeviceProp_t prop;
        if (hipGetDeviceProperties(&prop, d->device) == hipSuccess && prop.multiProcessorCount > 0) c->cfg.num_cus = prop.multiProcessorCount;
    }
    rc = build_topology(c, d); if (rc) return rc;
    rc = decide_policy(c, d, long_chain); if (rc) return rc;
    local_dof_terms(c);
    c->thermo.global_terms = c->thermo.local_terms;
    c->d.mass = nullptr; c->d.pair_drude = c->d.pair_parent = c->d.group = c->d.resid = nullptr;
    c->d.constraint_i = c->d.constraint_j = nullptr;

    if (!host_only) {
        rc = allocate(c); if (rc) return rc;
        rc = resident_census(c); if (rc) return rc;
    }
    rc = finalize_thermostat(c); if (rc) return rc;
    *out = owner.release();
    return TGNH_OK;
}

extern "C" tgnh_status tgnh_destroy(tgnh_handle h) {
    CHECK_H(h);
    if (h->xchg.rccl_comm) (void)tgnh_rccl_shutdown(h);
    if (!h->host_only) (void)hipSetDevice(h->device);
    delete h;
    return TGNH_OK;
}

extern "C" tgnh_status tgnh_bind_buffers(tgnh_handle h, void* posq, void* posq_correction, void* velm,
                                         const void* force, void* pos_delta) {
    CHECK_H(h);
    if (h->host_only) return fail(TGNH_ERR_STATE, "host-only handle (device -1): no GPU work can be launched on it");
    if (!posq || !velm || !force) return fail(TGNH_ERR_ARG, "posq, velm and force are required");
    if (h->d.precision == TGNH_PREC_MIXED && !posq_correction) return fail(TGNH_ERR_ARG, "mixed precision needs posqCorrection");
    if ((h->owed.kick_pending || h->owed.end_pending) && (velm != h->bound.velm || force != h->bound.force))
        return fail(TGNH_ERR_STATE, "tgnh_bind_buffers: velm / force may not be rebound while a deferred half kick is pending (tgnh_flush first)");
    if (posq == h->bound.posq && posq_correction == h->bound.posq_corr && velm == h->bound.velm && force == h->bound.force && pos_delta == h->bound.pos_delta)
        return TGNH_OK;
    {
        HIP_OK(hipSetDevice(h->device));
        const size_t N = (size_t)h->d.num_particles, P = (size_t)h->d.padded_num_particles;
        const size_t r4 = h->d.precision == TGNH_PREC_DOUBLE ? 32 : 16, m4 = h->d.precision == TGNH_PREC_SINGLE ? 16 : 32;
        struct { const void* p; size_t need; const char* name; } bufs[] = {
            {posq, N * r4, "posq"}, {posq_correction, N * 16, "posqCorrection"}, {velm, N * m4, "velm"},
            {force, 3 * P * sizeof(long long), "force"}, {pos_delta, N * m4, "posDelta"}};
        for (const auto& b : bufs) {
            if (!b.p) continue;
            hipDeviceptr_t base = nullptr; size_t size = 0;
            if (hipMemGetAddressRange(&base, &size, const_cast<void*>(b.p)) != hipSuccess) { (void)hipGetLastError(); continue; }
            const size_t left = size - (size_t)(static_cast<const char*>(b.p) - static_cast<const char*>(base));
            if (left < b.need)
                return fail(TGNH_ERR_ARG, std::string("tgnh_bind_buffers: ") + b.name + " has " + std::to_string(left) + " bytes behind the pointer, the launches touch " + std::to_string(b.need));
        }
    }
    h->owed.ke_carry = false;
    h->bound.posq = posq; h->bound.posq_corr = posq_correction; h->bound.velm = velm; h->bound.force = force; h->bound.pos_delta = pos_delta;
    return TGNH_OK;
}

tgnh_status deferred_guard(tgnh_handle h, const char* what) {
    if (h->owed.first_half_done || h->owed.end_pending)
        return fail(TGNH_ERR_STATE, std::string(what) + ": not allowed between steps with TGNH_FLAG_DEFER_SCALE (the next thermostat half step has already run)");
    return TGNH_OK;
}

extern "C" tgnh_status tgnh_set_step_size(tgnh_handle h, double dt) {
    CHECK_H(h);
    if (!(dt > 0) || !std::isfinite(dt)) return fail(TGNH_ERR_ARG, "step size must be positive");
    if (dt != h->d.step_size) { tgnh_status rc = deferred_guard(h, "tgnh_set_step_size"); if (rc) return rc; }
    h->d.step_size = dt;
    return TGNH_OK;
}
extern "C" tgnh_status tgnh_set_drude_steps_per_real_step(tgnh_handle h, int n) {
    CHECK_H(h);
    if (n < 1) return fail(TGNH_ERR_ARG, "drudeStepsPerRealStep must be >= 1");
    if (n != h->d.drude_steps_per_real_step) { tgnh_status rc = deferred_guard(h, "tgnh_set_drude_steps_per_real_step"); if (rc) return rc; }
    h->d.drude_steps_per_real_step = n;
    return TGNH_OK;
}
extern "C" tgnh_status tgnh_set_max_drude_distance(tgnh_handle h, double dist) {
    CHECK_H(h);
    if (!(dist >= 0)) return fail(TGNH_ERR_ARG, "setMaxDrudeDistance: Distance cannot be negative");
    h->d.max_drude_distance = dist;
    return TGNH_OK;
}

extern "C" tgnh_status tgnh_get_local_dof_terms(tgnh_handle h, double* terms, int* count) {
    CHECK_H(h);
    if (count) *count = h->thermo.L.NT;
    if (terms) std::copy(h->thermo.local_terms.begin(), h->thermo.local_terms.end(), terms);
    return TGNH_OK;
}
extern "C" tgnh_status tgnh_set_global_dof_terms(tgnh_handle h, const double* terms, int count) {
    CHECK_H(h);
    if (!terms || count != h->thermo.L.NT) return fail(TGNH_ERR_ARG, "dof term count mismatch");
    if (h->run.step_count != 0) return fail(TGNH_ERR_STATE, "global dof must be set before the first step");
    if (!h->host_only) HIP_OK(hipSetDevice(h->device));
    h->thermo.global_terms.assign(terms, terms + count);
    return finalize_thermostat(h);
}
```

openmm_drudenose_amd/csrc/tgnh_step.cpp:

```cpp
#include "tgnh_host.h"

constexpr int64_t STATUS_POLL_EVERY = 64;

void note_status(tgnh_handle h, uint32_t flags) {
    if (h->status.failed_code) return;
    if (flags & 8u) {
        h->status.failed_code = TGNH_ERR_STATE;
        h->status.failed = "resident step (noticed at step " + std::to_string((long long)h->run.step_count) + "): the launch's work-groups did "
                    "not all become resident within the time limit (TGNH_FLAG_RESIDENT_STEP needs the device to itself)";
        if (flags & 4u) h->status.failed += "; the waiting work-groups timed out in turn (status bits 2 and 3)";
    } else if (flags & 16u) {
        h->status.failed_code = TGNH_ERR_STATE;
        h->status.failed = "kinetic-energy pass (noticed at step " + std::to_string((long long)h->run.step_count) + "): work-group 0 did not "
                    "receive every work-group's row of sums within the time limit (the sums were left as NaN: nothing integrated "
                    "on with a partial sum); the device is shared with something that keeps this launch's work-groups from running "
                    "-- or a chain was handed a NaN kinetic energy: with an all-reduce attached, the rank on which that happened";
    } else if (flags & 4u) {
        h->status.failed_code = TGNH_ERR_STATE;
        h->status.failed = "mailbox exchange timed out (noticed at step " + std::to_string((long long)h->run.step_count) +
                    "): a peer did not send its kinetic-energy sums; the run cannot continue";
    } else if ((flags & 1u) && h->d.mode == TGNH_MODE_DUALNH) {
        h->status.failed_code = TGNH_ERR_HARDWALL;
        h->status.failed = "Drude particle moved too far beyond hard wall constraint";
    }
// ... 201 lines not shown
        Timed t(h, s, kid);
        if (wave) HIP_OK(launch_wke(h->d.precision, ops, h->cfg.gb, a, grid, s));
        else HIP_OK(launch_tile(h->d.precision, ops, h->cfg.gb, a, grid, lds, s));
    }
    if (inline_chain) {
        h->owed.chain_ran(); h->owed.stage_pending = !pingpong;
    }
    if (h->cfg.alternate_sweeps) h->run.sweep_reverse ^= 1;
    return TGNH_OK;
}

ChainArgs chain_args(tgnh_handle h) {
    ChainArgs a{};
    a.L = h->thermo.L; a.st = h->thermo.d_state; a.partials = h->thermo.d_partials; a.nparts = h->run.ke_parts;
    a.nbig = h->topo.num_big;
    a.dt = h->d.step_size; a.S = h->d.drude_steps_per_real_step;
    a.dtc = a.dt / a.S; a.inv_dtc = 1.0 / a.dtc;
    a.realkbT = h->thermo.realkbT; a.drudekbT = h->thermo.drudekbT;
    a.lanes = 0;
#ifdef TGNH_TUNING
    if (const char* e = getenv("TGNH_CHAIN_LANES")) a.lanes = e[0] != '0';
#endif
    a.stage = h->thermo.d_stage;
    a.status = h->status.d_word;
    if (h->xchg.on) a.x = h->xchg.args;
    a.commit = h->owed.stage_pending ? 1 : 0;
    h->owed.stage_pending = false;
    return a;
}

static tgnh_status commit_stage(tgnh_handle h, hipStream_t s) {
    if (!h->owed.stage_pending) return TGNH_OK;
    ChainArgs a = chain_args(h);
    a.do_sum = 0; a.do_chain = 0;
    HIP_OK(launch_chain(a, s));
    return TGNH_OK;
}

static tgnh_status run_chain(tgnh_handle h, hipStream_t s, bool twice) {
    if (h->gather.chain) return run_chain_gather(h, s, false);
    ChainArgs a = chain_args(h);
    a.chain_twice = twice ? 1 : 0;
    if (h->xchg.on) {
        a.do_sum = 1; a.x_send = 1;
        if (h->cfg.inline_chain) {
            a.do_chain = 0;
            { Timed t(h, s, KID_CHAIN); HIP_OK(launch_chain(a, s)); }
            h->owed.chain_pending = true; h->owed.chain_pending_twice = twice; h->owed.xwait_pending = true;
        } else {
            a.do_chain = 1; a.x_wait = 1;
            Timed t(h, s, KID_CHAIN);
            HIP_OK(launch_chain(a, s));
        }
        return TGNH_OK;
    }
    if (h->cfg.inline_chain && !h->xchg.allreduce && h->thermo.L.NT <= CHAIN_INLINE_SUM_NT &&
        (h->run.ke_parts + h->topo.num_big <= h->cfg.inline_sum_rows || h->cfg.inline_sum_all)) {
        h->owed.chain_pending = true; h->owed.sum_pending = true; h->owed.chain_pending_twice = twice;
        return TGNH_OK;
    }
    const bool summed = h->owed.tail_summed;
    h->owed.tail_summed = false;
    if (h->cfg.inline_chain) {
        a.do_sum = 1; a.do_chain = 0;
        if (!summed) { Timed t(h, s, KID_CHAIN); HIP_OK(launch_chain(a, s)); }
        if (h->xchg.allreduce && h->xchg.allreduce(h->thermo.d_state + h->thermo.L.off_ke_red, h->thermo.L.NT, (void*)s, h->xchg.allreduce_user) != 0)
            return fail(TGNH_ERR_HIP, "all-reduce hook failed");
        h->owed.chain_pending = true; h->owed.chain_pending_twice = twice;
        return TGNH_OK;
    }
    if (h->xchg.allreduce) {
        a.do_sum = 1; a.do_chain = 0;
        if (!summed) { Timed t(h, s, KID_CHAIN); HIP_OK(launch_chain(a, s)); }
        if (h->xchg.allreduce(h->thermo.d_state + h->thermo.L.off_ke_red, h->thermo.L.NT, (void*)s, h->xchg.allreduce_user) != 0)
            return fail(TGNH_ERR_HIP, "all-reduce hook failed");
        a.do_sum = 0; a.do_chain = 1; a.commit = 0;
        { Timed t(h, s, KID_CHAIN); HIP_OK(launch_chain(a, s)); }
    } else {
        a.do_sum = summed ? 0 : 1; a.do_chain = 1;
        Timed t(h, s, KID_CHAIN);
        HIP_OK(launch_chain(a, s));
    }
    return TGNH_OK;
}

tgnh_status materialize_chain(tgnh_handle h, hipStream_t s) {
    { tgnh_status rc = settle_end(h, s); if (rc) return rc; }
    if (!h->owed.chain_pending) return commit_stage(h, s);
    ChainArgs a = chain_args(h);
    a.do_sum = h->owed.sum_pending ? 1 : 0; a.do_chain = 1; a.chain_twice = h->owed.chain_pending_twice ? 1 : 0;
    a.x_wait = h->owed.xwait_pending ? 1 : 0;
    a.ke_carry = h->owed.carry_pending ? 1 : 0;
    { Timed t(h, s, KID_CHAIN); HIP_OK(launch_chain(a, s)); }
    h->owed.chain_ran();
    return TGNH_OK;
}

static bool resident_kind(tgnh_handle h, int kind) {
    if (!((h->d.flags & TGNH_FLAG_RESIDENT_STEP) && h->cfg.inline_chain && h->cfg.gb != 0 && h->thermo.L.NT <= CHAIN_INLINE_SUM_NT &&
          (h->xchg.on || !h->xchg.allreduce))) return false;
    if (kind == 0 && h->cfg.wresident_per_cu > 0) return true;
    return h->cfg.resident_per_cu > 0 && h->thermo.L.C == 1;
}
bool resident_now(tgnh_handle h) {
    return resident_kind(h, (h->d.flags & TGNH_FLAG_DEFER_SCALE) ? 0 : 1);
}

extern "C" tgnh_status tgnh_get_step_path(tgnh_handle h, int* gather, const char** reason) {
    CHECK_H(h);
    if (gather) *gather = h->gather.generic ? (h->gather.chain ? 2 : 1) : 0;
    if (reason) *reason = h->gather.reason.c_str();
    return TGNH_OK;
}

extern "C" tgnh_status tgnh_get_resident_kernel(tgnh_handle h, int* which) {
    CHECK_H(h);
    if (!which) return fail(TGNH_ERR_ARG, "null out");
    const int kind = (h->d.flags & TGNH_FLAG_DEFER_SCALE) ? 0 : 1;
    *which = !resident_kind(h, kind) ? 0 : (kind == 0 && h->cfg.wresident_per_cu > 0) ? 2 : 1;
    return TGNH_OK;
}

static tgnh_status run_resident(tgnh_handle h, hipStream_t s, int kind) {
    if (h->owed.stage_pending) { tgnh_status rc = commit_stage(h, s); if (rc) return rc; }
    TileArgs a = tile_args(h, nullptr);
    const int ops2 = step_kind_ops2(kind);
    if ((ops2 & OP_POSDELTA) && !h->bound.pos_delta) return fail(TGNH_ERR_STATE, "posDelta buffer not bound");
    const bool hw = a.hardwall != 0 && (ops2 & (OP_DRIFT | OP_MOVE));
    const size_t lds = tile_lds_bytes(h->d.precision, ops2, hw, a.use_com != 0);
    int& grid = h->cfg.resident_grid[kind][hw ? 1 : 0];
    if (grid == 0 && !(kind == 0 && h->cfg.wresident_per_cu > 0)) {
        int per_cu = std::min(h->cfg.resident_per_cu, step_blocks_per_cu(h->d.precision, h->cfg.gb, kind, lds));
        if (per_cu < 1) return fail(TGNH_ERR_HIP, "step_kernel: occupancy query failed");
        grid = std::max(1, std::min(std::min(h->topo.num_tiles, per_cu * h->cfg.num_cus / h->cfg.resident_share), GRID_CAP));
    }
    a.chain_on = 1;
    a.chain = chain_args(h);
    a.chain.chain_twice = kind == 0 ? 1 : 0;
    a.chain.nparts = grid;
    a.x_wait = 1;
    if (!h->xchg.on) a.chain.x = h->meet.self_x;
    a.st_in = h->thermo.d_state; a.st_out = h->thermo.d_state;
    a.sync = h->meet.d_sync; a.rows = h->meet.d_rows;
    if (h->topo.num_big && a.use_com) { tgnh_status rc = run_big_com(h, kind == 0 || kind == 2, s); if (rc) return rc; }
    if (kind == 0 && h->cfg.wresident_per_cu > 0) {
        if (h->cfg.wresident_grid == 0) {
            const int need = (h->topo.num_wtiles + WBLOCK / 64 - 1) / (WBLOCK / 64);
            h->cfg.wresident_grid = std::max(1, std::min(std::min(need, h->cfg.wresident_per_cu * h->cfg.num_cus / h->cfg.resident_share), GRID_CAP));
        }
        a.chain.nparts = h->cfg.wresident_grid;
        h->run.ke_parts = h->cfg.wresident_grid;
        { tgnh_status rc = check_launch(h, a, h->cfg.wresident_grid, WBLOCK, true, true); if (rc) return rc; }
        Timed t(h, s, KID_STEP);
        HIP_OK(launch_wstep(h->d.precision, h->cfg.gb, h->thermo.L.C > 1, a, h->cfg.wresident_grid, s));
    } else {
        h->run.ke_parts = grid;
        { tgnh_status rc = check_launch(h, a, grid, TBLOCK, false, true); if (rc) return rc; }
        Timed t(h, s, KID_STEP);
        HIP_OK(launch_step(h->d.precision, h->cfg.gb, kind, a, grid, lds, s));
    }
    h->owed.resident_settled();
    return TGNH_OK;
}

static tgnh_status first_half(tgnh_handle h, hipStream_t s) {
    if (h->owed.first_half_done) return TGNH_OK;
    if (h->owed.ke_carry) {
        h->owed.ke_carry = false;
        if (h->topo.num_big && h->d.mode == TGNH_MODE_TGNH && h->d.use_com_temp_group) {
            tgnh_status rc = run_big_com(h, false, s); if (rc) return rc;
        }
        if (h->cfg.inline_chain) {
            h->owed.chain_pending = true; h->owed.chain_pending_twice = false; h->owed.sum_pending = false; h->owed.carry_pending = true;
            return TGNH_OK;
        }
        ChainArgs a = chain_args(h);
        a.do_sum = 0; a.do_chain = 1; a.ke_carry = 1;
        Timed t(h, s, KID_CHAIN);
        HIP_OK(launch_chain(a, s));
        return TGNH_OK;
    }
    tgnh_status rc = run_tile(h, OP_KE, KID_KE, s); if (rc) return rc;
    return run_chain(h, s, false);
}

tgnh_status entry(tgnh_handle h, bool need_bufs) {
    if (!h) return fail(TGNH_ERR_ARG, "null handle");
    h->owed.g_com_fresh = false;
    if (need_bufs) { tgnh_status rc = need_buffers(h); if (rc) return rc; }
    if (!h->host_only) {
        HIP_OK(hipSetDevice(h->device));
        if (h->status.h_seen) note_status(h, *h->status.h_seen);
    }
    if (h->status.failed_code) return fail(h->status.failed_code, h->status.failed);
    return TGNH_OK;
}

static tgnh_status poll_status_async(tgnh_handle h, hipStream_t s) {
    if (!h->status.h_seen || h->run.step_count % STATUS_POLL_EVERY != 0) return TGNH_OK;
    hipStreamCaptureStatus cs = hipStreamCaptureStatusNone;
    if (s != nullptr && hipStreamIsCapturing(s, &cs) == hipSuccess && cs != hipStreamCaptureStatusNone) return TGNH_OK;
    HIP_OK(hipMemcpyAsync(h->status.h_seen, h->status.d_word, sizeof(uint32_t), hipMemcpyDeviceToHost, s));
    return TGNH_OK;
}

static void start_of_step(tgnh_handle h) {
    if (h->cfg.alternate_sweeps) h->run.sweep_reverse = (int)(h->run.step_count & 1);
}

extern "C" tgnh_status tgnh_step_begin(tgnh_handle h, void* stream) {
    tgnh_status rc = entry(h, true); if (rc) return rc;
    hipStream_t s = (hipStream_t)stream;
    start_of_step(h);
    if (h->owed.end_pending) {
        if (resident_now(h)) return run_resident(h, s, 0);
        rc = settle_end(h, s); if (rc) return rc;
    }
    if (!(h->d.flags & TGNH_FLAG_DEFER_SCALE) && resident_now(h) && !h->owed.ke_carry)
        return run_resident(h, s, 1);
    rc = first_half(h, s); if (rc) return rc;
    rc = run_tile(h, (h->owed.kick_pending ? OP_PREKICK : 0) | OP_SCALE | OP_KICK | OP_DRIFT, KID_SKD, s); if (rc) return rc;
    h->owed.velocities_current(); h->owed.first_half_done = false;
    return TGNH_OK;
}

static tgnh_status second_half(tgnh_handle h, hipStream_t s, int kick_ops) {
    tgnh_status rc;
    const bool defer = (h->d.flags & TGNH_FLAG_DEFER_SCALE) != 0;
    h->owed.ke_carry = false;
    if (h->owed.scale_pending || h->owed.kick_pending || h->owed.end_pending) { rc = flush_impl(h, s); if (rc) return rc; }
    if (!defer && resident_now(h)) {
        rc = run_resident(h, s, kick_ops ? 2 : 4); if (rc) return rc;
        h->owed.ke_carry = h->cfg.carry_ok && !h->xchg.allreduce && !h->xchg.on;
        h->run.time += h->d.step_size;
        h->run.step_count += 1;
        return poll_status_async(h, s);
    }
    if (kick_ops && resident_now(h)) {
        h->owed.end_pending = true;
        h->run.time += h->d.step_size;
        h->run.step_count += 1;
        return poll_status_async(h, s);
    }
    const bool fold = !defer && kick_ops != 0 && !h->gather.generic;
    const int nostore = kick_ops && !h->gather.generic ? OP_NOSTORE : 0;
    h->owed.end_folded = fold;
    rc = run_tile(h, kick_ops | OP_KE | nostore, kick_ops ? KID_KICK_KE : KID_KE, s); if (rc) return rc;
    if (defer) {
        rc = run_chain(h, s, true); if (rc) return rc;
        h->owed.end_half_deferred(nostore != 0);
    } else {
        rc = run_chain(h, s, false); if (rc) return rc;
        rc = run_tile(h, (fold ? OP_PREKICK : 0) | OP_SCALE, KID_SCALE, s); if (rc) return rc;
        h->owed.ke_carry = h->cfg.carry_ok && !h->xchg.allreduce && !h->xchg.on;
    }
    h->run.time += h->d.step_size;
    h->run.step_count += 1;
    return poll_status_async(h, s);
}

extern "C" tgnh_status tgnh_step_end(tgnh_handle h, void* stream) {
    tgnh_status rc = entry(h, true); if (rc) return rc;
    return second_half(h, (hipStream_t)stream, OP_KICK);
}

tgnh_status settle_kick(tgnh_handle h, hipStream_t s) {
    return (h->owed.kick_pending || h->owed.end_pending) ? flush_impl(h, s) : TGNH_OK;
}

tgnh_status settle_end(tgnh_handle h, hipStream_t s) {
    if (!h->owed.end_pending) return TGNH_OK;
    h->owed.end_pending = false;
    tgnh_status rc = run_tile(h, OP_KICK | OP_KE | OP_NOSTORE, KID_KICK_KE, s); if (rc) return rc;
    rc = run_chain(h, s, true); if (rc) return rc;
    h->owed.end_half_deferred(true);
    return TGNH_OK;
}

extern "C" tgnh_status tgnh_step_begin_kick(tgnh_handle h, void* stream) {
    tgnh_status rc = entry(h, true); if (rc) return rc;
    hipStream_t s = (hipStream_t)stream;
    rc = settle_kick(h, s); if (rc) return rc;
    start_of_step(h);
    if (!(h->d.flags & TGNH_FLAG_DEFER_SCALE) && resident_now(h) && !h->owed.ke_carry) return run_resident(h, s, 3);
    rc = first_half(h, s); if (rc) return rc;
    rc = run_tile(h, OP_SCALE | OP_KICK | OP_POSDELTA, KID_OTHER, s); if (rc) return rc;
    h->owed.scale_pending = false; h->owed.first_half_done = false;
    return TGNH_OK;
}
extern "C" tgnh_status tgnh_step_begin_move(tgnh_handle h, void* stream) {
    tgnh_status rc = entry(h, true); if (rc) return rc;
    h->owed.ke_carry = false;
    rc = settle_kick(h, (hipStream_t)stream); if (rc) return rc;
    return run_tile(h, OP_MOVE, KID_OTHER, (hipStream_t)stream);
}
extern "C" tgnh_status tgnh_step_end_kick(tgnh_handle h, void* stream) {
    tgnh_status rc = entry(h, true); if (rc) return rc;
    h->owed.ke_carry = false;
    rc = settle_kick(h, (hipStream_t)stream); if (rc) return rc;
    return run_tile(h, OP_KICK, KID_OTHER, (hipStream_t)stream);
}
extern "C" tgnh_status tgnh_step_end_thermo(tgnh_handle h, void* stream) {
    tgnh_status rc = entry(h, true); if (rc) return rc;
    return second_half(h, (hipStream_t)stream, 0);
}
extern "C" tgnh_status tgnh_half_kick(tgnh_handle h, void* stream) { return tgnh_step_end_kick(h, stream); }

// ... 56 lines not shown
```

openmm_drudenose_amd/csrc/tgnh_tile_device.h:

```cpp
#ifndef TGNH_TILE_DEVICE_H_
#define TGNH_TILE_DEVICE_H_
#include "tgnh_internal.h"

namespace tgnh {
__device__ __forceinline__ double wave_sum(double v);
#ifdef TGNH_TRACE
static __device__ unsigned long long g_trace[GRID_CAP * 16];
#define TRACE(slot) do { if (threadIdx.x == 0 && (slot) < 16) g_trace[blockIdx.x * 16 + (slot)] = wall_clock64(); } while (0)
#define TRACE_WAIT() __builtin_amdgcn_s_waitcnt(0)
#define TGNH_TRACE_READERS(read_name, clear_name)                                                            \
    extern "C" int read_name(unsigned long long* out) {                                                      \
        return (int)hipMemcpyFromSymbol(out, HIP_SYMBOL(tgnh::g_trace), sizeof(unsigned long long) * tgnh::GRID_CAP * 16); \
    }                                                                                                        \
    extern "C" int clear_name() {                                                                            \
        void* p = nullptr;                                                                                   \
        if (hipGetSymbolAddress(&p, HIP_SYMBOL(tgnh::g_trace)) != hipSuccess) return 1;                      \
        return (int)hipMemset(p, 0, sizeof(unsigned long long) * tgnh::GRID_CAP * 16);                       \
    }
static __device__ __attribute__((unused)) unsigned long long g_chain_trace[8];
#define CHAIN_TRACE(slot) do { if (threadIdx.x == 0) { g_chain_trace[2 * (slot)] = wall_clock64(); g_chain_trace[2 * (slot) + 1] = clock64(); } } while (0)
#else
#define TRACE(slot) do {} while (0)
#define TRACE_WAIT() do {} while (0)
#define CHAIN_TRACE(slot) do {} while (0)
#endif
}
#include "tgnh_chain_device.h"

namespace tgnh {

template <int PREC> struct Prec;
template <> struct Prec<TGNH_PREC_SINGLE> { typedef float real; typedef float mixed; typedef float4 real4; typedef float4 mixed4; };
template <> struct Prec<TGNH_PREC_MIXED>  { typedef float real; typedef double mixed; typedef float4 real4; typedef double4 mixed4; };
template <> struct Prec<TGNH_PREC_DOUBLE> { typedef double real; typedef double mixed; typedef double4 real4; typedef double4 mixed4; };

__device__ __forceinline__ float4 mk4(float x, float y, float z, float w) { return make_float4(x, y, z, w); }
__device__ __forceinline__ double4 mk4(double x, double y, double z, double w) { return make_double4(x, y, z, w); }
__device__ __forceinline__ float rcp_(float x) { return 1.0f / x; }
__device__ __forceinline__ double rcp_(double x) {
    double r = __builtin_amdgcn_rcp(x);
    r = fma(fma(-x, r, 1.0), r, r);
    r = fma(fma(-x, r, 1.0), r, r);
    return r;
}
__device__ __forceinline__ float sqrt_(float x) { return sqrtf(x); }
__device__ __forceinline__ double sqrt_(double x) { return sqrt(x); }
__device__ __forceinline__ float abs_(float x) { return fabsf(x); }
__device__ __forceinline__ double abs_(double x) { return fabs(x); }

#ifndef TGNH_WAVE_SUM_DPP
#define TGNH_WAVE_SUM_DPP 1
#endif
template <int CTRL, int ROW_MASK>
__device__ __forceinline__ double dpp_add(const double v) {
    const int lo = __builtin_amdgcn_update_dpp(0, __double2loint(v), CTRL, ROW_MASK, 0xf, false);
    const int hi = __builtin_amdgcn_update_dpp(0, __double2hiint(v), CTRL, ROW_MASK, 0xf, false);
    return v + __hiloint2double(hi, lo);
}
__device__ __forceinline__ double wave_sum(double v) {
#if TGNH_WAVE_SUM_DPP
    v = dpp_add<0xb1, 0xf>(v);
    v = dpp_add<0x4e, 0xf>(v);
    v = dpp_add<0x114, 0xf>(v);
    v = dpp_add<0x118, 0xf>(v);
    v = dpp_add<0x142, 0xa>(v);
    v = dpp_add<0x143, 0xc>(v);
    return __hiloint2double(__builtin_amdgcn_readlane(__double2hiint(v), 63), __builtin_amdgcn_readlane(__double2loint(v), 63));
#else
#pragma unroll
    for (int off = 32; off > 0; off >>= 1) v += __shfl_xor(v, off, 64);
    return v;
#endif
}


template <int PREC, int GB> struct TileEnv {
    typedef typename Prec<PREC>::mixed mixed;
    typedef typename Prec<PREC>::mixed4 mixed4;
    static constexpr bool SOA = sizeof(mixed) == 8;
    static constexpr int GBR = GB > 0 ? GB : 1;
    mixed4* sv;
    mixed4* scom;
    mixed4* sx;
    double* s_scale;
    double* wbins0;
    char* smem;
    int tid, G;
    bool use_com;
    mixed dt, fscale, s_com, s_drude;
    double ke_g[GBR], ke_com, ke_drude;
    __device__ __forceinline__ static void st_img(mixed4* img, int i, const mixed4& u) {
        mixed* imgc = reinterpret_cast<mixed*>(img);
        if (SOA) { imgc[i] = u.x; imgc[TILE_SLOTS + i] = u.y; imgc[2 * TILE_SLOTS + i] = u.z; imgc[3 * TILE_SLOTS + i] = u.w; }
        else img[i] = u;
    }
    __device__ __forceinline__ static mixed4 ld_img(const mixed4* img, int i) {
        const mixed* imgc = reinterpret_cast<const mixed*>(img);
        if (SOA) return mk4(imgc[i], imgc[TILE_SLOTS + i], imgc[2 * TILE_SLOTS + i], imgc[3 * TILE_SLOTS + i]);
        return img[i];
    }
    __device__ __forceinline__ void init(const TileArgs& a, char* smem_, double* s_scale_, bool hardwall_lds) {
        smem = smem_; s_scale = s_scale_;
        sv = reinterpret_cast<mixed4*>(smem); scom = sv + TILE_SLOTS; sx = scom + TILE_RES;
        tid = threadIdx.x; G = a.num_groups; use_com = a.use_com != 0;
        dt = (mixed)a.dt;
        fscale = (mixed)(0.5 * a.dt / 4294967296.0);
        s_com = 1; s_drude = 1;
        wbins0 = reinterpret_cast<double*>(sx + (hardwall_lds ? TILE_SLOTS : 0));
        clear_ke();
    }
    __device__ __forceinline__ void clear_ke() {
#pragma unroll
        for (int b = 0; b < GBR; b++) ke_g[b] = 0.0;
        ke_com = 0.0; ke_drude = 0.0;
        if (GB == 0) { double* w = wbins0 + (tid >> 6) * G; for (int g = tid & 63; g < G; g += 64) w[g] = 0.0; }
    }
};

__device__ __forceinline__ size_t row_word(const int r, const int j) {
    return ((size_t)(r >> 6) * (2 * CHAIN_INLINE_SUM_NT) + j) * 64 + (r & 63);
}

template <int PREC, int GB, bool TAGGED, int NTH = TBLOCK>
__device__ __forceinline__ void ke_reduce(const TileArgs& a, TileEnv<PREC, GB>& e, const unsigned tag = 0u, double* scratch = nullptr) {
    typedef TileEnv<PREC, GB> E;
    const int tid = e.tid, G = e.G;
    double (&ke_g)[E::GBR] = e.ke_g;
    double ke_com = e.ke_com, ke_drude = e.ke_drude;
    auto put = [&](const int b, double v) {
        if (TAGGED) {
            unsigned long long* cell = a.rows + row_word((int)blockIdx.x, 2 * b);
            const unsigned long long bits = (unsigned long long)__double_as_longlong(v), t = (unsigned long long)tag << 32;
            __hip_atomic_store(cell, t | (bits & 0xffffffffull), __ATOMIC_RELAXED, __HIP_MEMORY_SCOPE_SYSTEM);
            __hip_atomic_store(cell + 64, t | (bits >> 32), __ATOMIC_RELAXED, __HIP_MEMORY_SCOPE_SYSTEM);
        } else a.partials[(size_t)blockIdx.x * (G + 2) + b] = v;
    };
    double* sred = scratch ? scratch : reinterpret_cast<double*>(e.smem);
    const int lane = tid & 63, wv = tid >> 6;
#pragma unroll
    for (int b = 0; b < GB; b++) ke_g[b] = wave_sum(ke_g[b]);
    if (GB == 0) __syncthreads();
    ke_com = wave_sum(ke_com);
    ke_drude = wave_sum(ke_drude);
    if (lane == 0) {
#pragma unroll
        for (int b = 0; b < GB; b++) sred[wv * (GB + 2) + b] = ke_g[b];
        sred[wv * (GB + 2) + GB] = ke_com;
        sred[wv * (GB + 2) + GB + 1] = ke_drude;
    }
    __syncthreads();
    if (tid < GB + 2) {
        double s = 0.0;
#pragma unroll
        for (int w = 0; w < NTH / 64; w++) s += sred[w * (GB + 2) + tid];
// ... 40 lines not shown
        for (int r0 = tid; r0 < grid && ok; r0 += RB * NTH) {
#pragma unroll 1
            for (int b0 = 0; b0 < NT && ok; b0 += CH) {
                unsigned long long w[RB][2 * CH];
                bool have[RB];
#pragma unroll
                for (int k = 0; k < RB; k++) have[k] = r0 + k * NTH >= grid;
                unsigned n = 0;
                for (;;) {
#pragma unroll
                    for (int k = 0; k < RB; k++) {
                        if (!have[k]) {
                            const unsigned long long* cell = a.rows + row_word(r0 + k * NTH, 2 * b0);
#pragma unroll
                            for (int b = 0; b < 2 * CH; b++) if (b0 + b / 2 < NT) w[k][b] = xchg_ld(cell + b * 64);
                        }
                    }
                    bool all = true;
#pragma unroll
                    for (int k = 0; k < RB; k++) {
                        if (!have[k]) {
                            bool row = true;
#pragma unroll
                            for (int b = 0; b < 2 * CH; b++) if (b0 + b / 2 < NT) row = row && (w[k][b] >> 32) == want;
                            have[k] = row;
                        }
                        all = all && have[k];
                    }
                    if (all) break;
                    if (++n > XCHG_SPIN_LIMIT) { ok = false; break; }
                }
#pragma unroll
                for (int k = 0; k < RB; k++)
#pragma unroll
                    for (int b = 0; b < CH; b++)
                        if (b0 + b < NT && r0 + k * NTH < grid) {
                            const double v = __longlong_as_double((long long)((w[k][2 * b + 1] << 32) | (w[k][2 * b] & 0xffffffffull)));
#pragma unroll
                            for (int t = 0; t < NTM; t++) acc[t] += (t == b0 + b) ? v : 0.0;
                        }
            }
        }
    return ok;
}

struct MeetShared {
    double* s_scale;
    double (*s_part)[CHAIN_INLINE_SUM_NT];
    double* s_x;
    int* s_go_p; unsigned* s_gen_p; unsigned long long* s_seq1_p;
    const double* s_block;
};
template <int PREC, int GB, bool LEAN = false, int NTH = TBLOCK, bool MULTI = false, typename Prefetch>
__device__ __forceinline__ bool step_meet(const TileArgs& a, TileEnv<PREC, GB>& e, const unsigned gen0, const unsigned long long seq0,
                                          Chain1Regs& creg, const MeetShared& sh, Prefetch&& prefetch) {
    double* const s_scale = sh.s_scale; double (*const s_part)[CHAIN_INLINE_SUM_NT] = sh.s_part; double* const s_x = sh.s_x;
    int& s_go = *sh.s_go_p; unsigned& s_gen = *sh.s_gen_p; unsigned long long& s_seq1 = *sh.s_seq1_p;
    const int tid = threadIdx.x, G = a.num_groups, NT = G + 2, grid = (int)gridDim.x;
    const bool chain_wave = tid < 64, leader = blockIdx.x == 0;
    const int itg = tid & 63;
    const ChainLayout& L = a.chain.L;
    if (chain_wave) asm volatile("" :: "v"(creg.eta), "v"(creg.etaDot0), "v"(creg.etaDot1), "v"(creg.etaDotDot), "v"(creg.etaMass), "v"(creg.nkbt) : "memory");
    ke_reduce<PREC, GB, true, NTH>(a, e, gen0 + 1u, s_x);
    TRACE(2);
    prefetch();
    constexpr bool EARLY_PRE = PREC != TGNH_PREC_SINGLE && !LEAN;
    Chain1Pre cpre{};
    if (EARLY_PRE && chain_wave && !L.c1_quirk && !(MULTI && L.C > 1)) cpre = chain1_prepare(a.chain, creg, itg);

    if (tid == 0) { s_gen = gen0; s_seq1 = seq0 + 1ull; }
    __syncthreads();
    const unsigned long long want = (unsigned long long)(s_gen + 1u);
    if (leader) {
        unsigned long long* const my_peer = xchg_peer_of(a.chain.x, tid);
        constexpr int NTM = GB + 2;
        double acc[NTM];
#pragma unroll
        for (int b = 0; b < NTM; b++) acc[b] = 0.0;
        bool ok = true;
        TRACE(6);
        ok = collect_rows<GB, LEAN, NTH>(a, tid, grid, NT, want, acc);
        TRACE(10);
        if (!ok) {
            atomicOr(a.status, 8u);
            __hip_atomic_store(a.chain.x.dead, 1u, __ATOMIC_RELAXED, __HIP_MEMORY_SCOPE_AGENT);
        }
        const double* big = a.partials + (size_t)GRID_CAP * NT;
        for (int r = tid; r < a.chain.nbig; r += NTH)
#pragma unroll
            for (int b = 0; b < NTM; b++) if (b < NT) acc[b] += big[(size_t)r * NT + b];
#pragma unroll
        for (int b = 0; b < NTM; b++) {
            if (b < NT) {
                const double t = wave_sum(acc[b]);
                if ((tid & 63) == 0) s_part[tid >> 6][b] = t;
            }
        }
        const bool all_ok = __syncthreads_and(ok ? 1 : 0) != 0;
        TRACE(7);
        const XchgArgs& x = a.chain.x;
        const unsigned long long seq = s_seq1, stag = (seq & 0xffffffffull) << 32;
        if (tid == 0) { a.sync[1] = s_gen + 1u; *x.seq = seq; }
        const int tpp = NTH / x.world;
        if (all_ok && tid < tpp * x.world) {
            unsigned long long* const base = my_peer + xchg_cell(x, (unsigned)(seq & 1ull), x.rank, 0, 0);
            for (int q = tid / x.world; q < NT * XCHG_REPLICAS; q += tpp) {
                const int copy = q / NT, i = q - copy * NT;
                double v = 0.0;
#pragma unroll
                for (int w = 0; w < NTH / 64; w++) v += s_part[w][i];
                const unsigned long long bits = (unsigned long long)__double_as_longlong(v);
                unsigned long long* cell = base + (size_t)copy * XCHG_REPLICA_U64 + (size_t)i * XCHG_CELL_U64;
                __hip_atomic_store(cell, stag | (bits & 0xffffffffull), __ATOMIC_RELAXED, __HIP_MEMORY_SCOPE_SYSTEM);
                __hip_atomic_store(cell + 1, stag | (bits >> 32), __ATOMIC_RELAXED, __HIP_MEMORY_SCOPE_SYSTEM);
            }
        }
        TRACE(13);
    }
    if (chain_wave) {
        bool dead = false;
        const double mine = xchg_wait_sum<true>(a.chain.x, NT, itg, s_x + 64, seq0 + 1ull, &dead);
        TRACE(8);
        if (itg == 0) s_go = dead ? 0 : 1;
        if (!dead) {
            const bool write = leader;
            creg.ke = mine;
            if (write && itg < NT) a.st_out[L.off_ke_red + itg] = mine;
            if (write) {
                const double kesum = wave_sum(itg < NT ? mine : 0.0);
                if (itg == 63) a.st_out[L.off_kesum] = 0.5 * kesum;
            }
            if (MULTI && L.C > 1) chainN_run<false>(a.chain, sh.s_block, a.st_out, write, s_scale, itg, mine);
            else if (itg < NT) {
                if (L.c1_quirk) chain1q_run(a.chain, creg, a.st_out, write, s_scale, itg);
                else chain1_finish(a.chain, creg, EARLY_PRE ? cpre : chain1_prepare(a.chain, creg, itg), a.st_out, write, s_scale, itg);
            }
        }
    }
    __syncthreads();
    return s_go != 0;
}

template <int PREC> struct WStepIn {
    typename Prec<PREC>::mixed4 v;
    uint32_t meta;
    long long fx, fy, fz;
    typename Prec<PREC>::real4 p;
    float4 c;
    typename Prec<PREC>::mixed mass, cx, cy, cz;
};

struct WaveBounds { int ws, y, n; };

template <int PREC, int GB> struct WaveStep {
    typedef typename Prec<PREC>::real real;
    typedef typename Prec<PREC>::mixed mixed;
    typedef typename Prec<PREC>::real4 real4;
    typedef typename Prec<PREC>::mixed4 mixed4;
    const TileArgs& a;
    TileEnv<PREC, GB>* e;
    const double* s_scale;
    mixed *ix, *iy, *iz, *im, *jx, *jy, *jz;
    mixed4* __restrict__ velm; real4* __restrict__ posq; float4* __restrict__ pcorr;
    int lane, G, nw;
    bool use_com, hardwall;
    mixed dt, fscale;
    PatternWord pw;
    __device__ __forceinline__ WaveStep(const TileArgs& a_, TileEnv<PREC, GB>* e_, const double* s_scale_, mixed* img, const int lane_)
        : a(a_), e(e_), s_scale(s_scale_), ix(img), iy(img + WAVE_SLOTS), iz(img + 2 * WAVE_SLOTS), im(img + 3 * WAVE_SLOTS),
          jx(img + 4 * WAVE_SLOTS), jy(img + 5 * WAVE_SLOTS), jz(img + 6 * WAVE_SLOTS),
          velm(reinterpret_cast<mixed4*>(a_.velm)), posq(reinterpret_cast<real4*>(a_.posq)), pcorr(reinterpret_cast<float4*>(a_.posq_corr)),
          lane(lane_), G(a_.num_groups), nw(a_.num_wtiles), use_com(a_.use_com != 0), hardwall(a_.hardwall != 0),
          dt((mixed)a_.dt), fscale((mixed)(0.5 * a_.dt / 4294967296.0)) {}
    __device__ __forceinline__ static void wfence() {
        __builtin_amdgcn_fence(__ATOMIC_RELEASE, "wavefront");
        __builtin_amdgcn_wave_barrier();
        __builtin_amdgcn_fence(__ATOMIC_ACQUIRE, "wavefront");
    }
    __device__ __forceinline__ void bounds(const int ww, WaveBounds& b) const {
        const int2* t = a.wave_tile + (a.reverse ? nw - 1 - ww : ww);
        b.ws = t[0].x; b.y = t[0].y; b.n = t[1].x - b.ws;
    }
    __device__ __forceinline__ void load_vf(const WaveBounds& b, WStepIn<PREC>& in) {
        const int idx = b.ws + lane;
        const bool patterned = pw.of(a, (uint32_t)b.y >> 8, lane);
        mixed4 v = mk4((mixed)0, (mixed)0, (mixed)0, (mixed)0);
        uint32_t meta = 64u << 10;
        long long fx = 0, fy = 0, fz = 0;
        if (lane < b.n) {
            v = reinterpret_cast<const mixed4*>(a.velm)[idx];
            if (!patterned) meta = a.wmeta[idx];
            fx = a.force[idx]; fy = a.force[idx + a.padded]; fz = a.force[idx + 2 * a.padded];
        }
        if (patterned && lane < b.n) meta = pw.word;
        in.v = v; in.meta = meta; in.fx = fx; in.fy = fy; in.fz = fz;
    }
    __device__ __forceinline__ void load_x(const WaveBounds& b, WStepIn<PREC>& in) const {
        const int idx = b.ws + lane;
        if (lane < b.n) {
            in.p = reinterpret_cast<const real4*>(a.posq)[idx];
            if (PREC == TGNH_PREC_MIXED) in.c = reinterpret_cast<const float4*>(a.posq_corr)[idx];
        }
    }
    template <bool KICK = true>
    __device__ __forceinline__ void prepare(WStepIn<PREC>& t, const WaveBounds& bd, const bool ke) {
        mixed4& v = t.v;
        const uint32_t m = t.meta;
        t.mass = v.w != 0 ? rcp_(v.w) : (mixed)0;
        if (KICK) {
            const mixed c = fscale * v.w;
            v.x += c * force_as(t.fx, (mixed)0);
            v.y += c * force_as(t.fy, (mixed)0);
            v.z += c * force_as(t.fz, (mixed)0);
        }
        ix[lane] = v.x; iy[lane] = v.y; iz[lane] = v.z; im[lane] = t.mass;
        wfence();
        mixed cx = 0, cy = 0, cz = 0;
        if (use_com) {
            const int j = (int)((m >> 17) & 63u), n1 = (int)((m >> 23) & 63u);
            const int first = lane - j;
            mixed px = 0, py = 0, pz = 0, pm = 0;
            for (int k = 0; k < (bd.y & 255); k++) {
                if (k <= n1) {
                    const mixed um = im[first + k];
                    px += ix[first + k] * um; py += iy[first + k] * um; pz += iz[first + k] * um; pm += um;
                }
            }
            const mixed wq = rcp_(pm);
            cx = px * wq; cy = py * wq; cz = pz * wq;
            if (ke && j == 0 && lane < bd.n)
                e->ke_com += ((double)cx * cx + (double)cy * cy + (double)cz * cz) * (double)pm;
        }
        t.cx = cx; t.cy = cy; t.cz = cz;
        if (ke) {
            const uint32_t role = m & 3u, g = (m >> 2) & 255u;
            const double rx = v.x - cx, ry = v.y - cy, rz = v.z - cz;
            double val = v.w != 0 ? (rx * rx + ry * ry + rz * rz) * (double)t.mass : 0.0;
            if (role == ROLE_DRUDE) {
                const int pl = lane + (int)((m >> 10) & 127u) - 64;
                const double dx = ix[pl] - v.x, dy = iy[pl] - v.y, dz = iz[pl] - v.z;
                const double mass1 = t.mass, mass2 = im[pl];
                const double mu = mass1 * mass2 * rcp_(mass1 + mass2);
                const double d = (dx * dx + dy * dy + dz * dz) * mu;
                e->ke_drude += d;
                val -= d;
            }
#pragma unroll
            for (int b = 0; b < GB; b++) e->ke_g[b] += (g == (uint32_t)b) ? val : 0.0;
        }
    }
    __device__ __forceinline__ void finish(WStepIn<PREC>& t, const WaveBounds& bd) {
        mixed4 v = t.v;
        const uint32_t m = t.meta;
        const uint32_t role = m & 3u, g = (m >> 2) & 255u;
        const int pl = lane + (int)((m >> 10) & 127u) - 64;
        const mixed mass = t.mass, cx = t.cx, cy = t.cy, cz = t.cz;
        const mixed s_com = (mixed)s_scale[G], s_drude = (mixed)s_scale[G + 1], s_g = (mixed)s_scale[g];
        mixed px = t.p.x, py = t.p.y, pz = t.p.z;
        const real pq = t.p.w;
        if (PREC == TGNH_PREC_MIXED) { px += (mixed)t.c.x; py += (mixed)t.c.y; pz += (mixed)t.c.z; }
        if (role == ROLE_NORMAL) {
            if (v.w != 0) {
                const mixed rx = v.x - cx, ry = v.y - cy, rz = v.z - cz;
                v.x = s_g * rx + s_com * (v.x - rx);
                v.y = s_g * ry + s_com * (v.y - ry);
                v.z = s_g * rz + s_com * (v.z - rz);
            }
        } else {
            const mixed ux = ix[pl], uy = iy[pl], uz = iz[pl], um = im[pl];
            const mixed rsx = v.x - cx, rsy = v.y - cy, rsz = v.z - cz;
            const mixed rpx = ux - cx, rpy = uy - cy, rpz = uz - cz;
            const mixed invTot = rcp_(mass + um);
            const mixed msf = invTot * mass, mpf = invTot * um;
            const mixed sdp = s_drude * mpf;
            v.x = s_g * (rsx * msf + rpx * mpf) + sdp * (rsx - rpx) + s_com * (v.x - rsx);
            v.y = s_g * (rsy * msf + rpy * mpf) + sdp * (rsy - rpy) + s_com * (v.y - rsy);
            v.z = s_g * (rsz * msf + rpz * mpf) + sdp * (rsz - rpz) + s_com * (v.z - rsz);
        }
        if (v.w != 0) {
            const mixed c = fscale * v.w;
            v.x += c * force_as(t.fx, (mixed)0);
            v.y += c * force_as(t.fy, (mixed)0);
            v.z += c * force_as(t.fz, (mixed)0);
            px += dt * v.x; py += dt * v.y; pz += dt * v.z;
        }
        if (hardwall) {
            wfence();
            ix[lane] = v.x; iy[lane] = v.y; iz[lane] = v.z;
            jx[lane] = px; jy[lane] = py; jz[lane] = pz;
            wfence();
            if (role != ROLE_NORMAL) {
                const mixed maxd = (mixed)a.max_dist, hws = (mixed)a.hw_scale;
                const mixed sxd = px - jx[pl], syd = py - jy[pl], szd = pz - jz[pl];
                const mixed d2 = sxd * sxd + syd * syd + szd * szd;
                if (d2 > maxd * maxd) {
                    const mixed4 uv = mk4(ix[pl], iy[pl], iz[pl], im[pl]);
                    const bool is_d = role == ROLE_DRUDE;
                    const mixed4 vel1 = is_d ? v : uv, vel2 = is_d ? uv : v;
                    const mixed dx = is_d ? sxd : -sxd, dy = is_d ? syd : -syd, dz = is_d ? szd : -szd;
                    const mixed r = sqrt_(d2);
                    const mixed rInv = rcp_(r);
                    if (rInv * maxd < (mixed)0.5) atomicOr(a.status, 1u);
                    const mixed bx = dx * rInv, by = dy * rInv, bz = dz * rInv;
                    const mixed mass1 = is_d ? mass : uv.w, mass2 = is_d ? uv.w : mass;
                    const mixed deltaR = r - maxd;
                    mixed deltaT = dt;
                    mixed dotvr1 = vel1.x * bx + vel1.y * by + vel1.z * bz;
                    const mixed vp1x = vel1.x - bx * dotvr1, vp1y = vel1.y - by * dotvr1, vp1z = vel1.z - bz * dotvr1;
                    const mixed invTot = rcp_(mass1 + mass2);
                    mixed dotvr2 = vel2.x * bx + vel2.y * by + vel2.z * bz;
                    const mixed vp2x = vel2.x - bx * dotvr2, vp2y = vel2.y - by * dotvr2, vp2z = vel2.z - bz * dotvr2;
                    const mixed vbCMass = (mass1 * dotvr1 + mass2 * dotvr2) * invTot;
                    dotvr1 -= vbCMass;
                    dotvr2 -= vbCMass;
                    if (dotvr1 != dotvr2) deltaT = deltaR / abs_(dotvr1 - dotvr2);
                    if (deltaT > dt) deltaT = dt;
                    const mixed vBond = hws / sqrt_(mass1);
                    dotvr1 = -dotvr1 * vBond * mass2 * invTot / abs_(dotvr1);
                    dotvr2 = -dotvr2 * vBond * mass1 * invTot / abs_(dotvr2);
                    const mixed dr1 = -deltaR * mass2 * invTot + deltaT * dotvr1;
                    const mixed dr2 = deltaR * mass1 * invTot + deltaT * dotvr2;
                    dotvr1 += vbCMass;
                    dotvr2 += vbCMass;
                    if (is_d) {
                        px += bx * dr1; py += by * dr1; pz += bz * dr1;
                        v.x = vp1x + bx * dotvr1; v.y = vp1y + by * dotvr1; v.z = vp1z + bz * dotvr1;
                    } else {
                        px += bx * dr2; py += by * dr2; pz += bz * dr2;
                        v.x = vp2x + bx * dotvr2; v.y = vp2y + by * dotvr2; v.z = vp2z + bz * dotvr2;
                    }
                }
            }
        }
        wfence();
        if (lane < bd.n) {
            const int idx = bd.ws + lane;
            velm[idx] = v;
            if (PREC == TGNH_PREC_MIXED) {
                const float hx = (float)px, hy = (float)py, hz = (float)pz;
                posq[idx] = mk4((real)hx, (real)hy, (real)hz, pq);
                pcorr[idx] = make_float4((float)(px - hx), (float)(py - hy), (float)(pz - hz), 0.0f);
            } else {
                posq[idx] = mk4((real)px, (real)py, (real)pz, pq);
            }
        }
    }
};

}
#endif
```

openmm_drudenose_amd/drudetgnhplugin.py:

```python
import ctypes as C

import numpy as np

from . import _lib
from ._lib import (MODE_DUALNH, MODE_TGNH, PREC_SINGLE, PREC_MIXED, PREC_DOUBLE,
                   FLAG_DEFER_SCALE, FLAG_RESIDENT_STEP, FLAG_WAVE_TILES, FLAG_TRUST_STATE_CHANGED, FLAG_GATHER)
from .synth import KB

_PREC = {"single": PREC_SINGLE, "mixed": PREC_MIXED, "double": PREC_DOUBLE}
_MODE = {"dualNH": MODE_DUALNH, "TGNH": MODE_TGNH}


class TgnhError(RuntimeError):

    def __init__(self, status, message):
        super().__init__(message)
        self.status = status


def _check(rc):
    if rc != _lib.TGNH_OK:
        raise TgnhError(rc, _lib.load().tgnh_last_error().decode())


# ... 13 lines not shown
        self._useCOMTempGroup = bool(useCOMTempGroup)
        self._constraintTolerance = 1e-5
        self._tempGroups = []
        self._particleTempGroup = []
        self._context = None

    def getTemperature(self): return self._temperature
    def setTemperature(self, temp): self._temperature = float(temp)
    def getCouplingTime(self): return self._couplingTime
    def setCouplingTime(self, tau): self._couplingTime = float(tau)
    def getDrudeTemperature(self): return self._drudeTemperature
    def setDrudeTemperature(self, temp): self._drudeTemperature = float(temp)
    def getDrudeCouplingTime(self): return self._drudeCouplingTime
    def setDrudeCouplingTime(self, tau): self._drudeCouplingTime = float(tau)
    def getMaxDrudeDistance(self): return self._maxDrudeDistance

    def setMaxDrudeDistance(self, distance):
        if distance < 0:
            raise TgnhError(_lib.ERR_ARG, "setMaxDrudeDistance: Distance cannot be negative")
        self._maxDrudeDistance = float(distance)
        if self._context is not None:
            self._context._push_scalars()

    def getStepSize(self): return self._stepSize

    def setStepSize(self, dt):
        self._stepSize = float(dt)
        if self._context is not None:
            self._context._push_scalars()

    def getConstraintTolerance(self): return self._constraintTolerance
    def setConstraintTolerance(self, tol): self._constraintTolerance = float(tol)
    def getDrudeStepsPerRealStep(self): return self._drudeSteps

    def setDrudeStepsPerRealStep(self, drudeSteps):
        self._drudeSteps = int(drudeSteps)
        if self._context is not None:
            self._context._push_scalars()

    def getNumNHChains(self): return self._numNHChains
    def setNumNHChains(self, numChains): self._numNHChains = int(numChains)
    def getUseDrudeNHChains(self): return int(self._useDrudeNHChains)
    def setUseDrudeNHChains(self, use): self._useDrudeNHChains = bool(use)
    def getUseCOMTempGroup(self): return int(self._useCOMTempGroup)
    def setUseCOMTempGroup(self, use): self._useCOMTempGroup = bool(use)

    def getNumTempGroups(self): return len(self._tempGroups)

    def addTempGroup(self):
        self._tempGroups.append(len(self._tempGroups))
        return len(self._tempGroups) - 1

    def addParticleTempGroup(self, tempGroup):
        if not 0 <= tempGroup < len(self._tempGroups):
            raise TgnhError(_lib.ERR_ARG, "Index out of range")
        if not isinstance(self._particleTempGroup, list):
            self._particleTempGroup = [int(x) for x in self._particleTempGroup]
        self._particleTempGroup.append(int(tempGroup))
        return len(self._particleTempGroup) - 1

    def setParticleTempGroup(self, particle, tempGroup):
        if not 0 <= particle < len(self._particleTempGroup) or not 0 <= tempGroup < len(self._tempGroups):
            raise TgnhError(_lib.ERR_ARG, "Index out of range")
        self._particleTempGroup[particle] = int(tempGroup)

    def getParticleTempGroup(self, particle):
        if not 0 <= particle < len(self._particleTempGroup):
            raise TgnhError(_lib.ERR_ARG, "Index out of range")
        return int(self._particleTempGroup[particle])

    def step(self, steps):
        if self._context is None:
            raise TgnhError(_lib.ERR_STATE, "This Integrator is not bound to a context!")
        self._context.step(steps)

    def computeKineticEnergy(self):
        return self._context.kinetic_energy()

    def _resolve_groups(self, num_particles):
        if len(self._particleTempGroup) == 0:
            if len(self._tempGroups) == 0:
                self._tempGroups.append(0)
            self._particleTempGroup = np.zeros(num_particles, np.int32)
        elif len(self._particleTempGroup) != num_particles:
            raise TgnhError(_lib.ERR_ARG, "Number of particles assigned with temperature groups does not match the number of system particles")
        return np.asarray(self._particleTempGroup, np.int32), len(self._tempGroups)


def create_handle(lib, system, integrator, group, ngroups, mode, precision, device, flags, kB, padded):
    n = system.num_particles
    d = _lib.TgnhDesc()
    d.struct_size = C.sizeof(_lib.TgnhDesc)
    d.mode, d.precision, d.flags, d.device = mode, precision, int(flags), device
    d.num_particles, d.padded_num_particles = n, padded
    d.num_pairs, d.num_groups, d.num_residues = system.num_pairs, ngroups, system.num_residues
    d.num_constraints = len(system.constraints)
    d.has_cm_motion_remover = int(system.has_cm_motion_remover)
    group = np.ascontiguousarray(group, np.int32)
    ci = np.ascontiguousarray(system.constraints[:, 0]) if len(system.constraints) else None
    cj = np.ascontiguousarray(system.constraints[:, 1]) if len(system.constraints) else None
    d.mass = system.mass.ctypes.data_as(_lib.c_f64p)
    d.pair_drude = system.pair_drude.ctypes.data_as(_lib.c_i32p)
    d.pair_parent = system.pair_parent.ctypes.data_as(_lib.c_i32p)
    d.group = group.ctypes.data_as(_lib.c_i32p)
    d.resid = system.resid.ctypes.data_as(_lib.c_i32p)
    if ci is not None:
        d.constraint_i = ci.ctypes.data_as(_lib.c_i32p)
        d.constraint_j = cj.ctypes.data_as(_lib.c_i32p)
    d.kB = kB
    d.temperature, d.coupling_time = integrator.getTemperature(), integrator.getCouplingTime()
    d.drude_temperature, d.drude_coupling_time = integrator.getDrudeTemperature(), integrator.getDrudeCouplingTime()
    d.step_size = integrator.getStepSize()
    d.drude_steps_per_real_step = integrator.getDrudeStepsPerRealStep()
    d.num_nh_chains = integrator.getNumNHChains()
    d.use_drude_nh_chains = integrator.getUseDrudeNHChains()
    d.use_com_temp_group = integrator.getUseCOMTempGroup()
    d.max_drude_distance = integrator.getMaxDrudeDistance()
    h = C.c_void_p()
    _check(lib.tgnh_create(C.byref(d), C.byref(h)))
    return h


class _HandleQueries:

    def _stream(self):
        return None

    def step_path(self):
        g, why = C.c_int(), C.c_char_p()
        _check(self.lib.tgnh_get_step_path(self.h, C.byref(g), C.byref(why)))
        return ("tiled", "gather", "gather")[g.value], (why.value or b"").decode()

    def local_dof_terms(self):
        n = C.c_int()
        _check(self.lib.tgnh_get_local_dof_terms(self.h, None, C.byref(n)))
        out = np.zeros(n.value)
        _check(self.lib.tgnh_get_local_dof_terms(self.h, out.ctypes.data_as(_lib.c_f64p), C.byref(n)))
        return out

    def set_global_dof_terms(self, total):
        total = np.ascontiguousarray(total, np.float64)
        _check(self.lib.tgnh_set_global_dof_terms(self.h, total.ctypes.data_as(_lib.c_f64p), len(total)))

    def num_thermostats(self):
        n = C.c_int()
        _check(self.lib.tgnh_get_num_thermostats(self.h, C.byref(n)))
        return n.value

    def dof(self):
        n = self.num_thermostats()
        dof, nkt = np.zeros(n), np.zeros(n)
        _check(self.lib.tgnh_get_dof(self.h, dof.ctypes.data_as(_lib.c_f64p), nkt.ctypes.data_as(_lib.c_f64p)))
        return dof, nkt

    def thermostat_state(self, which):
        n = C.c_int()
        _check(self.lib.tgnh_get_thermostat_len(self.h, which, C.byref(n)))
        out = np.zeros(n.value)
        _check(self.lib.tgnh_get_thermostat_state(self.h, which, self._stream(), out.ctypes.data_as(_lib.c_f64p)))
        return out

    def set_thermostat_state(self, which, arr):
        arr = np.ascontiguousarray(arr, np.float64)
        _check(self.lib.tgnh_set_thermostat_state(self.h, which, self._stream(), arr.ctypes.data_as(_lib.c_f64p)))

    def topology(self, which):
        n = C.c_int()
        _check(self.lib.tgnh_get_topology_len(self.h, which, C.byref(n)))
        out = np.zeros(n.value, np.int32)
        _check(self.lib.tgnh_get_topology(self.h, which, out.ctypes.data_as(_lib.c_i32p)))
        return out


class HostTopology(_HandleQueries):

    def __init__(self, system, integrator, mode="TGNH", precision="mixed", flags=0, kB=KB):
        self.lib = _lib.load()
        group, ngroups = integrator._resolve_groups(system.num_particles)
        self.group, self.num_groups = group, ngroups
        n = system.num_particles
        self.h = create_handle(self.lib, system, integrator, group, ngroups, _MODE[mode], _PREC[precision], -1, flags, kB,
                               (n + 31) // 32 * 32)

    def close(self):
        if getattr(self, "h", None):
            self.lib.tgnh_destroy(self.h)
            self.h = None

    def __del__(self):
        try:
            self.close()
        except Exception:
            pass


class HipContext(_HandleQueries):

    def __init__(self, system, integrator, mode="TGNH", precision="mixed", device=0, flags=0, kB=KB,
                 k_drude=None, k_tether=None, allreduce=None, global_dof_sum=None, lattice_sites=True):
        import torch
        self.torch = torch
        self.lib = _lib.load()
        if not torch.cuda.is_available():
            raise RuntimeError("the DrudeTGNH HIP path needs a GPU (torch.cuda.is_available() is False); there is no CPU fallback")
        self.system, self.integrator = system, integrator
        self.mode, self.precision = _MODE[mode], _PREC[precision]
        self.dev = torch.device("cuda", device)
        n = system.num_particles
        self.n = n
        self.padded = (n + 31) // 32 * 32
        group, ngroups = integrator._resolve_groups(n)
        self.group, self.num_groups = group, ngroups
        from .synth import K_DRUDE, K_TETHER
        self.k_drude = K_DRUDE if k_drude is None else k_drude
        self.k_tether = K_TETHER if k_tether is None else k_tether

        with torch.cuda.device(self.dev):
            h = create_handle(self.lib, system, integrator, group, ngroups, self.mode, self.precision, device, flags, kB,
                              self.padded)
        self.h = h
        self._hook = None
        if global_dof_sum is not None:
            self.set_global_dof_terms(global_dof_sum(self.local_dof_terms()))
        if allreduce is not None:
            self.set_allreduce(allreduce)

        rdt = torch.float32 if self.precision != PREC_DOUBLE else torch.float64
        mdt = torch.float32 if self.precision == PREC_SINGLE else torch.float64
        self.rdt, self.mdt = rdt, mdt
        self.posq = torch.zeros((n, 4), dtype=rdt, device=self.dev)
        self.posq_corr = torch.zeros((n, 4), dtype=torch.float32, device=self.dev) if self.precision == PREC_MIXED else None
        self.velm = torch.zeros((n, 4), dtype=mdt, device=self.dev)
        self.force = torch.zeros(3 * self.padded, dtype=torch.int64, device=self.dev)
        self.pos_delta = torch.zeros((n, 4), dtype=mdt, device=self.dev)
        self.x0 = torch.zeros((n, 4), dtype=rdt, device=self.dev)
        self.sites_packed = False
        self.unpacked_sites = False
        self.use_lattice_sites = bool(lattice_sites)
        inv = np.where(system.mass == 0.0, 0.0, 1.0 / np.where(system.mass == 0.0, 1.0, system.mass))
        self.velm[:, 3] = torch.from_numpy(inv).to(self.dev, mdt)
        _check(self.lib.tgnh_bind_buffers(self.h, self.posq.data_ptr(),
                                          self.posq_corr.data_ptr() if self.posq_corr is not None else None,
                                          self.velm.data_ptr(), self.force.data_ptr(), self.pos_delta.data_ptr()))
        integrator._context = self
        self.force_fn = None
        self.state_hook = None
        self.ke_sum_valid = False
        self.constrained = False
        if system.cluster_atoms is not None and len(system.cluster_atoms):
            _check(self.lib.tgnh_harness_set_clusters(self.h, len(system.cluster_atoms),
                                                      system.cluster_atoms.ctypes.data_as(_lib.c_i32p),
                                                      system.cluster_dist.ctypes.data_as(_lib.c_f64p)))
            self.constrained = True
        if system.site_atoms is not None and len(system.site_atoms):
            _check(self.lib.tgnh_harness_set_virtual_sites(self.h, len(system.site_atoms),
                                                           system.site_atoms.ctypes.data_as(_lib.c_i32p),
                                                           system.site_weights.ctypes.data_as(_lib.c_f64p)))
            self.constrained = True
        if system.positions is not None:
            self.setPositions(system.positions)
            self.set_sites(system.positions)
        if system.velocities is not None:
            self.setVelocities(system.velocities)
        if system.positions is not None:
            self.compute_forces()

    def _stream(self):
        return C.c_void_p(self.torch.cuda.current_stream(self.dev).cuda_stream)

    def _push_scalars(self):
        i = self.integrator
        _check(self.lib.tgnh_set_step_size(self.h, i.getStepSize()))
        _check(self.lib.tgnh_set_drude_steps_per_real_step(self.h, i.getDrudeStepsPerRealStep()))
        _check(self.lib.tgnh_set_max_drude_distance(self.h, i.getMaxDrudeDistance()))

    def close(self):
        if getattr(self, "h", None):
            self.torch.cuda.synchronize(self.dev)
            self.lib.tgnh_destroy(self.h)
            self.h = None

    def __del__(self):
        try:
            self.close()
        except Exception:
            pass

    def set_allreduce(self, fn):
        torch = self.torch

        def _hook(buf, count, stream, user):
            try:
                t = self._ke_view(buf, count)
                fn(t)
                return 0
            except Exception as e:
                print("all-reduce hook failed:", e)
                return 1
        self._hook = _lib.ALLREDUCE_FN(_hook)
        self._views = {}
        _check(self.lib.tgnh_set_allreduce(self.h, self._hook, None))

    RCCL_ID_BYTES = 128

    def rccl_init(self, world, rank, unique_id):
        _check(self.lib.tgnh_rccl_init(self.h, int(world), int(rank), C.c_char_p(unique_id)))
# ... 337 lines not shown
```

Measured before the change: 4334 steps/s.

## Add cache-residency plan using nontemporal loads/stores in resident wave step kernel

Adds a residency planner that compares per-particle state bytes against an assumed 256 MiB Infinity Cache. When the state does not fit, it selects a wave-step kernel variant that uses nontemporal loads and stores for positions and corrections, so velocity and force data are more likely to stay cached between the two passes. A lead fraction of tiles can also use nontemporal velocity/force loads in pass 1, though the default policy bits leave that off. The risk is that streaming hints evict useful lines or lower occupancy; the census now takes the smaller of the two kernels' blocks-per-CU.

```diff
diff --git a/include/drude_tgnh.h b/include/drude_tgnh.h
--- a/include/drude_tgnh.h
+++ b/include/drude_tgnh.h
@@ -97,6 +97,8 @@
 tgnh_status tgnh_get_resident_work_groups(tgnh_handle h, int* per_compute_unit);
 tgnh_status tgnh_get_step_path(tgnh_handle h, int* gather, const char** reason);
 tgnh_status tgnh_get_resident_kernel(tgnh_handle h, int* which);
+tgnh_status tgnh_get_residency_plan(tgnh_handle h, int64_t out[4]);
+tgnh_status tgnh_set_cache_bytes(tgnh_handle h, int64_t bytes);
 
 #define TGNH_XCHG_HANDLE_BYTES 64
 tgnh_status tgnh_exchange_create(tgnh_handle h, int world, int rank, void* ipc_handle_out, void** mailbox_out);
diff --git a/openmm_drudenose_amd/_lib.py b/openmm_drudenose_amd/_lib.py
--- a/openmm_drudenose_amd/_lib.py
+++ b/openmm_drudenose_amd/_lib.py
@@ -56,6 +56,8 @@
     "tgnh_set_resident_share": (C.c_int, [C.c_void_p, C.c_int]),
     "tgnh_get_resident_work_groups": (C.c_int, [C.c_void_p, C.POINTER(C.c_int)]),
     "tgnh_get_resident_kernel": (C.c_int, [C.c_void_p, C.POINTER(C.c_int)]),
+    "tgnh_get_residency_plan": (C.c_int, [C.c_void_p, C.POINTER(C.c_int64)]),
+    "tgnh_set_cache_bytes": (C.c_int, [C.c_void_p, C.c_int64]),
     "tgnh_get_step_path": (C.c_int, [C.c_void_p, C.POINTER(C.c_int), C.POINTER(C.c_char_p)]),
     "tgnh_exchange_create": (C.c_int, [C.c_void_p, C.c_int, C.c_int, C.c_void_p, C.POINTER(C.c_void_p)]),
     "tgnh_exchange_attach": (C.c_int, [C.c_void_p, C.c_char_p]),
diff --git a/openmm_drudenose_amd/csrc/tgnh_context.h b/openmm_drudenose_amd/csrc/tgnh_context.h
--- a/openmm_drudenose_amd/csrc/tgnh_context.h
+++ b/openmm_drudenose_amd/csrc/tgnh_context.h
@@ -97,6 +97,10 @@
         int resident_grid[5][2] = {{0, 0}, {0, 0}, {0, 0}, {0, 0}, {0, 0}};
         int resident_share = 1;
         int wresident_per_cu = 0, wresident_grid = 0;
+        long long cache_bytes = tgnh::INFINITY_CACHE_BYTES;
+        long long state_bytes = 0;
+        bool wplan = false;
+        int wnt_lead = 0;
         int resident_per_cu = 0;
     } cfg;
     struct Owed {
diff --git a/openmm_drudenose_amd/csrc/tgnh_internal.h b/openmm_drudenose_amd/csrc/tgnh_internal.h
--- a/openmm_drudenose_amd/csrc/tgnh_internal.h
+++ b/openmm_drudenose_amd/csrc/tgnh_internal.h
@@ -29,6 +29,9 @@
 
 constexpr int WAVE_SLOTS = 64;
 constexpr int WBLOCK = 512;
+enum : int { WNT_P1_V = 1, WNT_P1_F = 2, WNT_P2_V = 4, WNT_P2_F = 8, WNT_X = 16, WNT_C = 32, WNT_ST_V = 64, WNT_ST_X = 128, WNT_ST_C = 256 };
+constexpr long long INFINITY_CACHE_BYTES = 256ll << 20;
+constexpr int CACHE_RESIDENT_PERCENT = 90;
 inline uint32_t pack_wmeta(uint32_t role, uint32_t group, int partner_off, uint32_t pos_in_mol, uint32_t mol_slots_m1) {
     return role | (group << 2) | ((uint32_t)(partner_off + 64) << 10) | (pos_in_mol << 17) | (mol_slots_m1 << 23);
 }
@@ -132,6 +135,7 @@
     uint32_t* status;
     unsigned int* sync;
     int census;
+    int wnt_lead;
     unsigned long long* rows;
     const int2* wave_tile;
     const uint32_t* wmeta;
@@ -216,8 +220,9 @@
 hipError_t launch_step(int precision, int gb, int kind, const TileArgs& a, int grid, size_t lds, hipStream_t s);
 int step_blocks_per_cu(int precision, int gb, int kind, size_t lds);
 int step_kind_ops2(int kind);
-hipError_t launch_wstep(int precision, int gb, bool multi, const TileArgs& a, int grid, hipStream_t s);
-int wstep_blocks_per_cu(int precision, int gb, bool multi);
+hipError_t launch_wstep(int precision, int gb, bool multi, bool plan, const TileArgs& a, int grid, hipStream_t s);
+int wstep_blocks_per_cu(int precision, int gb, bool multi, bool plan);
+int wstep_plan_bits();
 hipError_t launch_wke(int precision, int ops, int gb, const TileArgs& a, int grid, hipStream_t s);
 int wke_blocks_per_cu(int precision, int ops, int gb);
 hipError_t launch_chain(const ChainArgs& a, hipStream_t s);
diff --git a/openmm_drudenose_amd/csrc/tgnh_kernels.hip b/openmm_drudenose_amd/csrc/tgnh_kernels.hip
--- a/openmm_drudenose_amd/csrc/tgnh_kernels.hip
+++ b/openmm_drudenose_amd/csrc/tgnh_kernels.hip
@@ -820,105 +820,19 @@
 
 template <int PREC, int GB, bool MULTI = false>
 __global__ __launch_bounds__(WBLOCK) void wstep_kernel(const TileArgs a) {
-    typedef typename Prec<PREC>::mixed mixed;
-    static_assert(GB > 0, "register bins only");
-    __shared__ double s_scale[MAX_GROUPS + 2];
-    __shared__ double s_part[WBLOCK / 64][CHAIN_INLINE_SUM_NT];
-    __shared__ double s_x[64 + XCHG_MAX_WORLD * CHAIN_INLINE_SUM_NT];
-    __shared__ int s_go;
-    __shared__ unsigned s_gen;
-    __shared__ unsigned long long s_seq1;
-    __shared__ mixed s_img[WBLOCK / 64][7][WAVE_SLOTS];
-    __shared__ double s_block[256];
-    const int tid = threadIdx.x, lane = tid & 63, G = a.num_groups, NT = G + 2;
-    const int wv = __builtin_amdgcn_readfirstlane(tid >> 6);
-    const bool chain_wave = tid < 64;
-    const int itg = tid & 63;
-    if (a.census) {
-        if (tid == 0) {
-            __hip_atomic_fetch_add(&a.sync[2], 1u, __ATOMIC_RELAXED, __HIP_MEMORY_SCOPE_AGENT);
-            unsigned n = 0;
-            while (__hip_atomic_load(&a.sync[2], __ATOMIC_RELAXED, __HIP_MEMORY_SCOPE_AGENT) < gridDim.x && ++n < CENSUS_SPIN_LIMIT)
-                __builtin_amdgcn_s_sleep(16);
-            if (__hip_atomic_load(&a.sync[2], __ATOMIC_RELAXED, __HIP_MEMORY_SCOPE_AGENT) < gridDim.x) atomicOr(&a.sync[3], 1u);
-        }
-        return;
-    }
-    TileEnv<PREC, GB> e;
-    e.tid = tid; e.G = G; e.smem = nullptr; e.wbins0 = nullptr; e.s_scale = s_scale;
-    e.clear_ke();
-    WaveStep<PREC, GB> ws(a, &e, s_scale, &s_img[wv][0][0], lane);
-    typedef WaveBounds Bounds;
-    auto bounds = [&](const int ww, Bounds& b) { ws.bounds(ww, b); };
-    auto load_vf = [&](const Bounds& b, WStepIn<PREC>& in) { ws.load_vf(b, in); };
-    auto load_x = [&](const Bounds& b, WStepIn<PREC>& in) { ws.load_x(b, in); };
-    auto prepare = [&](WStepIn<PREC>& t, const Bounds& bd, const bool ke) { ws.template prepare<true>(t, bd, ke); };
-    auto finish = [&](WStepIn<PREC>& t, const Bounds& bd) { ws.finish(t, bd); };
-    auto wfence = [] { WaveStep<PREC, GB>::wfence(); };
-
-    unsigned gen0 = 0;
-    unsigned long long seq0 = 0;
-    Chain1Regs creg{};
-    if (chain_wave) {
-        gen0 = __hip_atomic_load(&a.sync[1], __ATOMIC_RELAXED, __HIP_MEMORY_SCOPE_AGENT);
-        seq0 = __hip_atomic_load(a.chain.x.seq, __ATOMIC_RELAXED, __HIP_MEMORY_SCOPE_AGENT);
-        if (itg < NT && !(MULTI && a.chain.L.C > 1)) creg = chain1_load(a.chain, a.st_in, itg);
-    }
-    if (MULTI && a.chain.L.C > 1 && tid < a.chain.L.total) s_block[tid] = a.st_in[tid];
-
-    const int nw = a.num_wtiles, stride = (int)gridDim.x * (WBLOCK / 64);
-
-    TRACE(0);
-    const int w0 = __builtin_amdgcn_readfirstlane((int)blockIdx.x * (WBLOCK / 64) + wv);
-    const bool have = w0 < nw;
-    int w = w0;
-    Bounds b0{}, b1{};
-    WStepIn<PREC> cur;
-    if (have) {
-        bounds(w, b0);
-        if (w + stride < nw) bounds(w + stride, b1);
-        load_vf(b0, cur);
-    }
-    while (have) {
-#ifdef TGNH_TRACE
-        if (w == w0) { asm volatile("s_waitcnt vmcnt(0)" ::: "memory"); TRACE(3); }
+    constexpr int POLICY = 0;
+#include "tgnh_wstep_body.h"
+}
+
+#ifndef TGNH_WSTEP_PLAN
+#define TGNH_WSTEP_PLAN (WNT_X | WNT_C | WNT_ST_X | WNT_ST_C)
 #endif
-        prepare(cur, b0, true);
-#ifdef TGNH_TRACE
-        if (w == w0) TRACE(4);
-#endif
-        if (w + stride >= nw) break;
-        wfence();
-        w += stride;
-        b0 = b1;
-        if (w + stride < nw) bounds(w + stride, b1);
-        load_vf(b0, cur);
-    }
-    const int w_last = w;
-    TRACE(1);
-    MeetShared sh{s_scale, s_part, s_x, &s_go, &s_gen, &s_seq1, s_block};
-    if (!step_meet<PREC, GB, true, WBLOCK, MULTI>(a, e, gen0, seq0, creg, sh, [&] {
-            if (have) {
-                load_x(b0, cur);
-                if (w_last - stride >= 0) bounds(w_last - stride, b1);
-            }
-        })) return;
-
-    TRACE(9);
-    if (have) {
-        w = w_last;
-        finish(cur, b0);
-        TRACE(5);
-        while (w - stride >= 0) {
-            w -= stride;
-            b0 = b1;
-            if (w - stride >= 0) bounds(w - stride, b1);
-            load_vf(b0, cur); load_x(b0, cur);
-            prepare(cur, b0, false);
-            finish(cur, b0);
-        }
-    }
-    TRACE(15);
+constexpr int WSTEP_PLAN = TGNH_WSTEP_PLAN;
+template <int PREC, int GB>
+__global__ __launch_bounds__(WBLOCK) void wstep_plan_kernel(const TileArgs a) {
+    constexpr int POLICY = WSTEP_PLAN;
+    constexpr bool MULTI = false;
+#include "tgnh_wstep_body.h"
 }
 
 constexpr int CHAIN_LDS_DOUBLES = 2048;
@@ -1377,8 +1291,17 @@
 template <int PREC, bool MULTI> static step_fn_t wstep_fn_gb(int gb) {
     return gb <= 1 ? wstep_kernel<PREC, 1, MULTI> : gb <= 4 ? wstep_kernel<PREC, 4, MULTI> : wstep_kernel<PREC, 8, MULTI>;
 }
-static step_fn_t wstep_fn(int precision, int gb, bool multi) {
-    if (gb == 0) return nullptr;
+template <int PREC> static step_fn_t wstep_plan_fn_gb(int gb) {
+    return gb <= 1 ? wstep_plan_kernel<PREC, 1> : gb <= 4 ? wstep_plan_kernel<PREC, 4> : wstep_plan_kernel<PREC, 8>;
+}
+static step_fn_t wstep_fn(int precision, int gb, bool multi, bool plan = false) {
+    if (gb == 0 || (plan && multi)) return nullptr;
+    if (plan) switch (precision) {
+        case TGNH_PREC_SINGLE: return wstep_plan_fn_gb<TGNH_PREC_SINGLE>(gb);
+        case TGNH_PREC_MIXED: return wstep_plan_fn_gb<TGNH_PREC_MIXED>(gb);
+        case TGNH_PREC_DOUBLE: return wstep_plan_fn_gb<TGNH_PREC_DOUBLE>(gb);
+        default: return nullptr;
+    }
     switch (precision) {
         case TGNH_PREC_SINGLE: return multi ? wstep_fn_gb<TGNH_PREC_SINGLE, true>(gb) : wstep_fn_gb<TGNH_PREC_SINGLE, false>(gb);
         case TGNH_PREC_MIXED: return multi ? wstep_fn_gb<TGNH_PREC_MIXED, true>(gb) : wstep_fn_gb<TGNH_PREC_MIXED, false>(gb);
@@ -1386,14 +1309,15 @@
         default: return nullptr;
     }
 }
-hipError_t launch_wstep(int precision, int gb, bool multi, const TileArgs& a, int grid, hipStream_t s) {
-    step_fn_t fn = wstep_fn(precision, gb, multi);
+int wstep_plan_bits() { return WSTEP_PLAN; }
+hipError_t launch_wstep(int precision, int gb, bool multi, bool plan, const TileArgs& a, int grid, hipStream_t s) {
+    step_fn_t fn = wstep_fn(precision, gb, multi, plan);
     if (!fn) return hipErrorInvalidValue;
     TGNH_LAUNCH(fn, dim3(grid), dim3(WBLOCK), 0, s, a);
     return hipGetLastError();
 }
-int wstep_blocks_per_cu(int precision, int gb, bool multi) {
-    step_fn_t fn = wstep_fn(precision, gb, multi);
+int wstep_blocks_per_cu(int precision, int gb, bool multi, bool plan) {
+    step_fn_t fn = wstep_fn(precision, gb, multi, plan);
     int n = 0;
     if (!fn || hipOccupancyMaxActiveBlocksPerMultiprocessor(&n, reinterpret_cast<const void*>(fn), WBLOCK, 0) != hipSuccess) return 0;
     return n;
diff --git a/openmm_drudenose_amd/csrc/tgnh_lifecycle.cpp b/openmm_drudenose_amd/csrc/tgnh_lifecycle.cpp
--- a/openmm_drudenose_amd/csrc/tgnh_lifecycle.cpp
+++ b/openmm_drudenose_amd/csrc/tgnh_lifecycle.cpp
@@ -132,6 +132,37 @@
     return TGNH_OK;
 }
 
+static void plan_residency(tgnh_context* c) {
+    const int prec = c->d.precision;
+    const int v = prec == TGNH_PREC_SINGLE ? 16 : 32, x = prec == TGNH_PREC_DOUBLE ? 32 : 16, corr = prec == TGNH_PREC_MIXED ? 16 : 0, f = 24;
+#ifdef TGNH_TUNING
+    if (const char* e = getenv("TGNH_CACHE_BYTES")) c->cfg.cache_bytes = std::max(1ll, atoll(e));
+#endif
+    const double slots = (double)c->d.num_particles, cache = (double)c->cfg.cache_bytes;
+    c->cfg.state_bytes = (long long)c->d.num_particles * (v + x + corr + f);
+    c->cfg.wplan = (double)c->cfg.state_bytes * 100.0 > cache * CACHE_RESIDENT_PERCENT && c->thermo.L.C == 1 && c->topo.num_wtiles > 0;
+    const double vf = slots * (v + f);
+    c->cfg.wnt_lead = c->cfg.wplan && vf > cache ? (int)((double)c->topo.num_wtiles * (1.0 - cache / vf)) : 0;
+#ifdef TGNH_TUNING
+    if (const char* e = getenv("TGNH_WPLAN")) c->cfg.wplan = c->cfg.wplan && e[0] != '0';
+    if (const char* e = getenv("TGNH_WNT_LEAD_PERMILLE")) c->cfg.wnt_lead = c->cfg.wplan ? (int)((long long)c->topo.num_wtiles * atoi(e) / 1000) : 0;
+#endif
+}
+
+extern "C" tgnh_status tgnh_set_cache_bytes(tgnh_handle h, int64_t bytes) {
+    CHECK_H(h);
+    if (bytes < 1) return fail(TGNH_ERR_ARG, "cache size must be positive");
+    h->cfg.cache_bytes = bytes;
+    plan_residency(h);
+    return TGNH_OK;
+}
+extern "C" tgnh_status tgnh_get_residency_plan(tgnh_handle h, int64_t out[4]) {
+    CHECK_H(h);
+    if (!out) return fail(TGNH_ERR_ARG, "null out");
+    out[0] = h->cfg.wplan ? wstep_plan_bits() : 0; out[1] = h->cfg.wnt_lead; out[2] = h->cfg.state_bytes; out[3] = h->cfg.cache_bytes;
+    return TGNH_OK;
+}
+
 static tgnh_status resident_census(tgnh_context* c) {
     if (!(c->d.flags & TGNH_FLAG_RESIDENT_STEP) || c->cfg.gb == 0 || !c->cfg.inline_chain || c->thermo.L.NT > CHAIN_INLINE_SUM_NT) return TGNH_OK;
     const int kind = (c->d.flags & TGNH_FLAG_DEFER_SCALE) ? 0 : 1;
@@ -146,8 +177,10 @@
 #ifdef TGNH_TUNING
     if (const char* e = getenv("TGNH_WSTEP")) want_w = want_w && e[0] != '0';
 #endif
-    return census(c, want_w ? wstep_blocks_per_cu(c->d.precision, c->cfg.gb, multi) : 0,
-                  [&](const TileArgs& a, int grid) { return launch_wstep(c->d.precision, c->cfg.gb, multi, a, grid, (hipStream_t)0); },
+    int per_cu = want_w ? wstep_blocks_per_cu(c->d.precision, c->cfg.gb, multi, false) : 0;
+    if (want_w && !multi) per_cu = std::min(per_cu, wstep_blocks_per_cu(c->d.precision, c->cfg.gb, false, true));
+    return census(c, per_cu,
+                  [&](const TileArgs& a, int grid) { return launch_wstep(c->d.precision, c->cfg.gb, multi, false, a, grid, (hipStream_t)0); },
                   &c->cfg.wresident_per_cu);
 }
 
@@ -180,6 +213,7 @@
     }
     rc = build_topology(c, d); if (rc) return rc;
     rc = decide_policy(c, d, long_chain); if (rc) return rc;
+    plan_residency(c);
     local_dof_terms(c);
     c->thermo.global_terms = c->thermo.local_terms;
     c->d.mass = nullptr; c->d.pair_drude = c->d.pair_parent = c->d.group = c->d.resid = nullptr;
diff --git a/openmm_drudenose_amd/csrc/tgnh_step.cpp b/openmm_drudenose_amd/csrc/tgnh_step.cpp
--- a/openmm_drudenose_amd/csrc/tgnh_step.cpp
+++ b/openmm_drudenose_amd/csrc/tgnh_step.cpp
@@ -377,7 +377,8 @@
         h->run.ke_parts = h->cfg.wresident_grid;
         { tgnh_status rc = check_launch(h, a, h->cfg.wresident_grid, WBLOCK, true, true); if (rc) return rc; }
         Timed t(h, s, KID_STEP);
-        HIP_OK(launch_wstep(h->d.precision, h->cfg.gb, h->thermo.L.C > 1, a, h->cfg.wresident_grid, s));
+        a.wnt_lead = h->cfg.wnt_lead;
+        HIP_OK(launch_wstep(h->d.precision, h->cfg.gb, h->thermo.L.C > 1, h->cfg.wplan, a, h->cfg.wresident_grid, s));
     } else {
         h->run.ke_parts = grid;
         { tgnh_status rc = check_launch(h, a, grid, TBLOCK, false, true); if (rc) return rc; }
diff --git a/openmm_drudenose_amd/csrc/tgnh_tile_device.h b/openmm_drudenose_amd/csrc/tgnh_tile_device.h
--- a/openmm_drudenose_amd/csrc/tgnh_tile_device.h
+++ b/openmm_drudenose_amd/csrc/tgnh_tile_device.h
@@ -1,5 +1,6 @@
 #ifndef TGNH_TILE_DEVICE_H_
 #define TGNH_TILE_DEVICE_H_
+#include <type_traits>
 #include "tgnh_internal.h"
 
 namespace tgnh {
@@ -346,7 +347,21 @@
 
 struct WaveBounds { int ws, y, n; };
 
-template <int PREC, int GB> struct WaveStep {
+template <typename T4> __device__ __forceinline__ T4 nt_load(const T4* p) {
+    typedef typename std::remove_cv<decltype(T4::x)>::type S;
+    typedef S __attribute__((ext_vector_type(4))) V;
+    const V u = __builtin_nontemporal_load(reinterpret_cast<const V*>(p));
+    T4 r; r.x = u.x; r.y = u.y; r.z = u.z; r.w = u.w;
+    return r;
+}
+template <typename T4> __device__ __forceinline__ void nt_store(T4* p, const T4& v) {
+    typedef typename std::remove_cv<decltype(T4::x)>::type S;
+    typedef S __attribute__((ext_vector_type(4))) V;
+    const V u = {v.x, v.y, v.z, v.w};
+    __builtin_nontemporal_store(u, reinterpret_cast<V*>(p));
+}
+
+template <int PREC, int GB, int POLICY = 0> struct WaveStep {
     typedef typename Prec<PREC>::real real;
     typedef typename Prec<PREC>::mixed mixed;
     typedef typename Prec<PREC>::real4 real4;
@@ -375,16 +390,27 @@
         const int2* t = a.wave_tile + (a.reverse ? nw - 1 - ww : ww);
         b.ws = t[0].x; b.y = t[0].y; b.n = t[1].x - b.ws;
     }
-    __device__ __forceinline__ void load_vf(const WaveBounds& b, WStepIn<PREC>& in) {
+    template <int PASS> __device__ __forceinline__ void load_vf(const WaveBounds& b, WStepIn<PREC>& in, const bool lead = false) {
+        constexpr bool NTV = (POLICY & (PASS == 1 ? WNT_P1_V : WNT_P2_V)) != 0, NTF = (POLICY & (PASS == 1 ? WNT_P1_F : WNT_P2_F)) != 0;
+        if constexpr (PASS == 1 && (NTV || NTF)) {
+            if (lead) load_vf_as<NTV, NTF>(b, in); else load_vf_as<false, false>(b, in);
+        } else load_vf_as<NTV, NTF>(b, in);
+    }
+    template <bool NTV, bool NTF> __device__ __forceinline__ void load_vf_as(const WaveBounds& b, WStepIn<PREC>& in) {
         const int idx = b.ws + lane;
         const bool patterned = pw.of(a, (uint32_t)b.y >> 8, lane);
         mixed4 v = mk4((mixed)0, (mixed)0, (mixed)0, (mixed)0);
         uint32_t meta = 64u << 10;
         long long fx = 0, fy = 0, fz = 0;
         if (lane < b.n) {
-            v = reinterpret_cast<const mixed4*>(a.velm)[idx];
+            if constexpr (NTV) v = nt_load(&reinterpret_cast<const mixed4*>(a.velm)[idx]);
+            else v = reinterpret_cast<const mixed4*>(a.velm)[idx];
             if (!patterned) meta = a.wmeta[idx];
-            fx = a.force[idx]; fy = a.force[idx + a.padded]; fz = a.force[idx + 2 * a.padded];
+            if constexpr (NTF) {
+                fx = __builtin_nontemporal_load(&a.force[idx]); fy = __builtin_nontemporal_load(&a.force[idx + a.padded]); fz = __builtin_nontemporal_load(&a.force[idx + 2 * a.padded]);
+            } else {
+                fx = a.force[idx]; fy = a.force[idx + a.padded]; fz = a.force[idx + 2 * a.padded];
+            }
         }
         if (patterned && lane < b.n) meta = pw.word;
         in.v = v; in.meta = meta; in.fx = fx; in.fy = fy; in.fz = fz;
@@ -392,8 +418,12 @@
     __device__ __forceinline__ void load_x(const WaveBounds& b, WStepIn<PREC>& in) const {
         const int idx = b.ws + lane;
         if (lane < b.n) {
-            in.p = reinterpret_cast<const real4*>(a.posq)[idx];
-            if (PREC == TGNH_PREC_MIXED) in.c = reinterpret_cast<const float4*>(a.posq_corr)[idx];
+            if constexpr ((POLICY & WNT_X) != 0) in.p = nt_load(&reinterpret_cast<const real4*>(a.posq)[idx]);
+            else in.p = reinterpret_cast<const real4*>(a.posq)[idx];
+            if (PREC == TGNH_PREC_MIXED) {
+                if constexpr ((POLICY & WNT_C) != 0) in.c = nt_load(&reinterpret_cast<const float4*>(a.posq_corr)[idx]);
+                else in.c = reinterpret_cast<const float4*>(a.posq_corr)[idx];
+            }
         }
     }
     template <bool KICK = true>
@@ -529,13 +559,15 @@
         wfence();
         if (lane < bd.n) {
             const int idx = bd.ws + lane;
-            velm[idx] = v;
+            constexpr bool NTV = (POLICY & WNT_ST_V) != 0, NTX = (POLICY & WNT_ST_X) != 0, NTC = (POLICY & WNT_ST_C) != 0;
+            if constexpr (NTV) nt_store(&velm[idx], v); else velm[idx] = v;
             if (PREC == TGNH_PREC_MIXED) {
                 const float hx = (float)px, hy = (float)py, hz = (float)pz;
-                posq[idx] = mk4((real)hx, (real)hy, (real)hz, pq);
-                pcorr[idx] = make_float4((float)(px - hx), (float)(py - hy), (float)(pz - hz), 0.0f);
+                if constexpr (NTX) nt_store(&posq[idx], mk4((real)hx, (real)hy, (real)hz, pq)); else posq[idx] = mk4((real)hx, (real)hy, (real)hz, pq);
+                if constexpr (NTC) nt_store(&pcorr[idx], make_float4((float)(px - hx), (float)(py - hy), (float)(pz - hz), 0.0f));
+                else pcorr[idx] = make_float4((float)(px - hx), (float)(py - hy), (float)(pz - hz), 0.0f);
             } else {
-                posq[idx] = mk4((real)px, (real)py, (real)pz, pq);
+                if constexpr (NTX) nt_store(&posq[idx], mk4((real)px, (real)py, (real)pz, pq)); else posq[idx] = mk4((real)px, (real)py, (real)pz, pq);
             }
         }
     }
diff --git a/openmm_drudenose_amd/csrc/tgnh_wstep_body.h b/openmm_drudenose_amd/csrc/tgnh_wstep_body.h
--- /dev/null
+++ b/openmm_drudenose_amd/csrc/tgnh_wstep_body.h
@@ -0,0 +1,100 @@
+    typedef typename Prec<PREC>::mixed mixed;
+    static_assert(GB > 0, "register bins only");
+    __shared__ double s_scale[MAX_GROUPS + 2];
+    __shared__ double s_part[WBLOCK / 64][CHAIN_INLINE_SUM_NT];
+    __shared__ double s_x[64 + XCHG_MAX_WORLD * CHAIN_INLINE_SUM_NT];
+    __shared__ int s_go;
+    __shared__ unsigned s_gen;
+    __shared__ unsigned long long s_seq1;
+    __shared__ mixed s_img[WBLOCK / 64][7][WAVE_SLOTS];
+    __shared__ double s_block[256];
+    const int tid = threadIdx.x, lane = tid & 63, G = a.num_groups, NT = G + 2;
+    const int wv = __builtin_amdgcn_readfirstlane(tid >> 6);
+    const bool chain_wave = tid < 64;
+    const int itg = tid & 63;
+    if (a.census) {
+        if (tid == 0) {
+            __hip_atomic_fetch_add(&a.sync[2], 1u, __ATOMIC_RELAXED, __HIP_MEMORY_SCOPE_AGENT);
+            unsigned n = 0;
+            while (__hip_atomic_load(&a.sync[2], __ATOMIC_RELAXED, __HIP_MEMORY_SCOPE_AGENT) < gridDim.x && ++n < CENSUS_SPIN_LIMIT)
+                __builtin_amdgcn_s_sleep(16);
+            if (__hip_atomic_load(&a.sync[2], __ATOMIC_RELAXED, __HIP_MEMORY_SCOPE_AGENT) < gridDim.x) atomicOr(&a.sync[3], 1u);
+        }
+        return;
+    }
+    TileEnv<PREC, GB> e;
+    e.tid = tid; e.G = G; e.smem = nullptr; e.wbins0 = nullptr; e.s_scale = s_scale;
+    e.clear_ke();
+    WaveStep<PREC, GB, POLICY> ws(a, &e, s_scale, &s_img[wv][0][0], lane);
+    typedef WaveBounds Bounds;
+    auto bounds = [&](const int ww, Bounds& b) { ws.bounds(ww, b); };
+    auto load_vf1 = [&](const int ww, const Bounds& b, WStepIn<PREC>& in) { ws.template load_vf<1>(b, in, ww < a.wnt_lead); };
+    auto load_vf2 = [&](const Bounds& b, WStepIn<PREC>& in) { ws.template load_vf<2>(b, in); };
+    auto load_x = [&](const Bounds& b, WStepIn<PREC>& in) { ws.load_x(b, in); };
+    auto prepare = [&](WStepIn<PREC>& t, const Bounds& bd, const bool ke) { ws.template prepare<true>(t, bd, ke); };
+    auto finish = [&](WStepIn<PREC>& t, const Bounds& bd) { ws.finish(t, bd); };
+    auto wfence = [] { WaveStep<PREC, GB, POLICY>::wfence(); };
+
+    unsigned gen0 = 0;
+    unsigned long long seq0 = 0;
+    Chain1Regs creg{};
+    if (chain_wave) {
+        gen0 = __hip_atomic_load(&a.sync[1], __ATOMIC_RELAXED, __HIP_MEMORY_SCOPE_AGENT);
+        seq0 = __hip_atomic_load(a.chain.x.seq, __ATOMIC_RELAXED, __HIP_MEMORY_SCOPE_AGENT);
+        if (itg < NT && !(MULTI && a.chain.L.C > 1)) creg = chain1_load(a.chain, a.st_in, itg);
+    }
+    if (MULTI && a.chain.L.C > 1 && tid < a.chain.L.total) s_block[tid] = a.st_in[tid];
+
+    const int nw = a.num_wtiles, stride = (int)gridDim.x * (WBLOCK / 64);
+
+    TRACE(0);
+    const int w0 = __builtin_amdgcn_readfirstlane((int)blockIdx.x * (WBLOCK / 64) + wv);
+    const bool have = w0 < nw;
+    int w = w0;
+    Bounds b0{}, b1{};
+    WStepIn<PREC> cur;
+    if (have) {
+        bounds(w, b0);
+        if (w + stride < nw) bounds(w + stride, b1);
+        load_vf1(w, b0, cur);
+    }
+    while (have) {
+#ifdef TGNH_TRACE
+        if (w == w0) { asm volatile("s_waitcnt vmcnt(0)" ::: "memory"); TRACE(3); }
+#endif
+        prepare(cur, b0, true);
+#ifdef TGNH_TRACE
+        if (w == w0) TRACE(4);
+#endif
+        if (w + stride >= nw) break;
+        wfence();
+        w += stride;
+        b0 = b1;
+        if (w + stride < nw) bounds(w + stride, b1);
+        load_vf1(w, b0, cur);
+    }
+    const int w_last = w;
+    TRACE(1);
+    MeetShared sh{s_scale, s_part, s_x, &s_go, &s_gen, &s_seq1, s_block};
+    if (!step_meet<PREC, GB, true, WBLOCK, MULTI>(a, e, gen0, seq0, creg, sh, [&] {
+            if (have) {
+                load_x(b0, cur);
+                if (w_last - stride >= 0) bounds(w_last - stride, b1);
+            }
+        })) return;
+
+    TRACE(9);
+    if (have) {
+        w = w_last;
+        finish(cur, b0);
+        TRACE(5);
+        while (w - stride >= 0) {
+            w -= stride;
+            b0 = b1;
+            if (w - stride >= 0) bounds(w - stride, b1);
+            load_vf2(b0, cur); load_x(b0, cur);
+            prepare(cur, b0, false);
+            finish(cur, b0);
+        }
+    }
+    TRACE(15);
diff --git a/openmm_drudenose_amd/drudetgnhplugin.py b/openmm_drudenose_amd/drudetgnhplugin.py
--- a/openmm_drudenose_amd/drudetgnhplugin.py
+++ b/openmm_drudenose_amd/drudetgnhplugin.py
@@ -189,6 +189,14 @@
         dof, nkt = np.zeros(n), np.zeros(n)
         _check(self.lib.tgnh_get_dof(self.h, dof.ctypes.data_as(_lib.c_f64p), nkt.ctypes.data_as(_lib.c_f64p)))
         return dof, nkt
+
+    def residency_plan(self):
+        out = (C.c_int64 * 4)()
+        _check(self.lib.tgnh_get_residency_plan(self.h, out))
+        return tuple(out)
+
+    def set_cache_bytes(self, nbytes):
+        _check(self.lib.tgnh_set_cache_bytes(self.h, int(nbytes)))
 
     def thermostat_state(self, which):
         n = C.c_int()
```

After: 4462 steps/s (median of 6 runs). 1.03x the previous value.
